# SinOncology/BreakID

Measured on AMD Instinct MI355X. Metric: M reads/s clustered+split-scanned, higher is better.
Workload: dtype int32/u8 (+f64 sd replay)

## Files before the change

### breakid_amd/csrc/api.hip

```cpp
#include <algorithm>
#include <cmath>
#include <limits>
#include <cstring>
#include <numeric>

#include "bk_common.h"
#include "prims.h"
#include "stream.h"
#include "join.h"
#include "cluster.h"
#include "bp.h"
#include "normal.h"
#include "genotype.h"
#include "clip.h"
#include "junction.h"
#include "evidence.h"
#include "unique.h"
#include "consensus.h"
#include "jfit.h"
#include "locsim.h"
#include "coverage.h"
#include "context.h"
#include "frame.h"
#include "link.h"
// ... 2250 lines not shown
int bk_debug_scan(bk_ctx *ctx, int elem_bytes, const void *in, uint64_t n, int in_place, void *out)
{
  return guarded(ctx, [&] {
    if (elem_bytes != 4 && elem_bytes != 8) throw bk_error(BK_ERR_ARG, "bk_debug_scan: elem_bytes must be 4 or 8");
    if (!out || (n && !in)) throw bk_error(BK_ERR_ARG, "bk_debug_scan: null argument");
    auto run = [&](auto zero) {
      using T = decltype(zero);
      T *d_in = ctx->dbg_in.as<T>(n + 1);
      T *d_out = in_place ? d_in : ctx->dbg_out.as<T>(n + 1);
      HIP_CHECK(hipMemsetAsync(d_out, 0xA5, (n + 1) * sizeof(T), ctx->st));
      if (n) HIP_CHECK(hipMemcpyAsync(d_in, in, n * sizeof(T), hipMemcpyHostToDevice, ctx->st));
      prims::exclusive_scan<T>(d_in, d_out, n, ctx->dbg_radix.scan_tmp, ctx->st);
      HIP_CHECK(hipMemcpyAsync(out, d_out, (n + 1) * sizeof(T), hipMemcpyDeviceToHost, ctx->st));
      HIP_CHECK(hipStreamSynchronize(ctx->st));
    };
    if (elem_bytes == 4)
      run(uint32_t(0));
    else
      run(uint64_t(0));
  });
}

int bk_debug_radix_sort(bk_ctx *ctx, const uint64_t *keys, const uint32_t *vals, uint64_t n, int begin_bit, int end_bit, uint64_t *keys_out, uint32_t *vals_out)
{
  return guarded(ctx, [&] {
    if (n && (!keys || !vals || !keys_out || !vals_out)) throw bk_error(BK_ERR_ARG, "bk_debug_radix_sort: null argument");
    if (begin_bit < 0 || end_bit > 64) throw bk_error(BK_ERR_ARG, "bk_debug_radix_sort: bits outside [0, 64]");
    prims::radix_check_count(n);
    if (!n) return;
    prims::RadixBufs &rb = ctx->dbg_radix;
    uint64_t *dk = ctx->dbg_in.as<uint64_t>(n);
    uint32_t *dv = ctx->dbg_vals.as<uint32_t>(n);
    HIP_CHECK(hipMemsetAsync(rb.keys_alt.as<uint64_t>(n), 0xA5, n * 8, ctx->st));
    HIP_CHECK(hipMemsetAsync(rb.vals_alt.as<uint32_t>(n), 0xA5, n * 4, ctx->st));
    HIP_CHECK(hipMemcpyAsync(dk, keys, n * 8, hipMemcpyHostToDevice, ctx->st));
    HIP_CHECK(hipMemcpyAsync(dv, vals, n * 4, hipMemcpyHostToDevice, ctx->st));
    uint64_t *ko = nullptr;
    uint32_t *vo = nullptr;
    prims::radix_sort_pairs(dk, dv, n, begin_bit, end_bit, rb, ctx->st, &ko, &vo);
    HIP_CHECK(hipMemcpyAsync(keys_out, ko, n * 8, hipMemcpyDeviceToHost, ctx->st));
    HIP_CHECK(hipMemcpyAsync(vals_out, vo, n * 4, hipMemcpyDeviceToHost, ctx->st));
    HIP_CHECK(hipStreamSynchronize(ctx->st));
  });
}

int bk_debug_prims_info(uint64_t out[4])
{
  if (!out) return BK_ERR_ARG;
  out[0] = prims::BLOCK;
  out[1] = prims::SCAN_TILE;
  out[2] = prims::SCAN_ONE_MAX;
  out[3] = prims::RS_TILE;
  return BK_OK;
}

int bk_sort_forms(bk_ctx *ctx, uint64_t out[3])
{
  return guarded(ctx, [&] {
    if (!out) throw bk_error(BK_ERR_ARG, "bk_sort_forms: null output");
    ctx->stage.sort_forms(out);
  });
}

int bk_debug_ahc(bk_ctx *ctx, const uint32_t *x, const uint32_t *y, uint32_t n, double w, uint32_t *idx_out, int32_t *cluster_out, uint32_t *n_out)
{
  return guarded(ctx, [&] {
    if (!x || !y || !idx_out || !cluster_out || !n_out) throw bk_error(BK_ERR_ARG, "bk_debug_ahc: null argument");
    std::vector<bk_pair> hp(n);
    for (uint32_t i = 0; i < n; ++i)
    {
      memset(&hp[i], 0, sizeof(bk_pair));
      hp[i].x = x[i];
      hp[i].y = y[i];
    }
    DevBuf dp, dcl;
    PairList L;
    L.n = n;
    L.ng = 1;
    std::vector<uint32_t> iota(n), gof(n, 0);
    std::iota(iota.begin(), iota.end(), 0u);
    uint64_t goff[2] = {0, n};
    HIP_CHECK(hipMemcpy(dp.as<bk_pair>(n + 1), hp.data(), n * sizeof(bk_pair), hipMemcpyHostToDevice));
    HIP_CHECK(hipMemcpy(L.idx.as<uint32_t>(n + 1), iota.data(), n * 4, hipMemcpyHostToDevice));
    HIP_CHECK(hipMemcpy(L.gof.as<uint32_t>(n + 1), gof.data(), n * 4, hipMemcpyHostToDevice));
    HIP_CHECK(hipMemcpy(L.goff.as<uint64_t>(2), goff, 16, hipMemcpyHostToDevice));
    ahc_cluster_all(dp.get<bk_pair>(), L, w, dcl, ctx->stage.ab, ctx->stage.cb(), ctx->st);
    *n_out = (uint32_t) L.n;
    if (L.n)
    {
      HIP_CHECK(hipMemcpyAsync(idx_out, L.idx.get<uint32_t>(), L.n * 4, hipMemcpyDeviceToHost, ctx->st));
      HIP_CHECK(hipMemcpyAsync(cluster_out, dcl.get<uint32_t>(), L.n * 4, hipMemcpyDeviceToHost, ctx->st));
    }
    HIP_CHECK(hipStreamSynchronize(ctx->st));
  });
}

}

namespace
{
struct FeedLink
{
  int device = 0, mapq_min = 20;
  bk_ctx *ctx = nullptr;
  int rc = BK_OK;
  std::string err;
  uint64_t done = 0;
  bool prepared = false, overflow = false;
  hipEvent_t t0 = nullptr, t1 = nullptr;
  template <class F> void guard(F &&f)
  {
    if (rc != BK_OK) return;
    try
    {
      f();
    }
    catch (const bk_error &e)
    {
      rc = e.code;
      err = e.msg;
    }
  }
};
void link_header(void *u, int nt, const char *const *names, const uint32_t *lens)
{
  FeedLink *L = (FeedLink *) u;
  if (L->ctx || L->rc != BK_OK) return;
  L->rc = bk_init(L->device, lens, names, nt, &L->ctx);
  if (L->rc != BK_OK) L->err = bk_last_error(nullptr);
}
void link_reset(void *u)
{
  FeedLink *L = (FeedLink *) u;
  L->guard([&] {
    if (L->ctx) HIP_CHECK(hipStreamSynchronize(L->ctx->st));
    L->done = 0;
    L->prepared = false;
    L->overflow = false;
  });
}
void link_before_move(void *u)
{
  FeedLink *L = (FeedLink *) u;
  L->guard([&] {
    if (L->ctx) HIP_CHECK(hipStreamSynchronize(L->ctx->st));
  });
}
void link_chunk(void *u, const bk_soa *cols, uint64_t n_ready, uint64_t n_est, hipEvent_t ready)
{
  FeedLink *L = (FeedLink *) u;
  L->guard([&] {
    bk_ctx *c = L->ctx;
    if (!c || n_ready < (uint64_t) STREAM_V + 1) return;
    c->rec = *cols;
    c->have_records = true;
    c->mapq_min = L->mapq_min;
    if (!L->prepared)
    {
      stream_prepare(c, n_est + n_est / 4);
      L->prepared = true;
    }
    const uint64_t lim = (n_ready - 1) / STREAM_V * STREAM_V;
    if (lim <= L->done) return;
    HIP_CHECK(hipStreamWaitEvent(c->st, ready, 0));
    StreamArgs a = stream_args(c, lim);
    a.q_begin = L->done / STREAM_V;
    launch_stream(a, c->st);
    L->done = lim;
  });
}
}


extern "C" {

int bk_bam_decode_device_ctx(const char *path, int device, int mapq_min, bk_bam_dev **bam_out, bk_ctx **ctx_out, int *n_targets, const char *const **names,
                             const uint32_t **lens, char *err, size_t errlen)
{
  auto fail = [&](int code, const std::string &m) {
    if (err && errlen) snprintf(err, errlen, "%s", m.c_str());
    return code;
  };
  if (!path || !bam_out || !ctx_out) return fail(BK_ERR_ARG, "bk_bam_decode_device_ctx: null argument");
  *bam_out = nullptr;
  *ctx_out = nullptr;
  FeedLink L;
  L.device = device;
  L.mapq_min = mapq_min;
  FeedConsumer fc;
  fc.user = &L;
  fc.on_header = link_header;
  fc.on_chunk = link_chunk;
  fc.before_move = link_before_move;
  fc.on_reset = link_reset;
  bk_soa cols;
  bk_bam_dev *bam = nullptr;
  int rc = bam_decode_device_impl(path, device, &bam, &cols, n_targets, names, lens, err, errlen, &fc);
  if (rc == BK_OK && L.rc != BK_OK) rc = fail(L.rc, L.err);
  if (rc == BK_OK && !L.ctx) rc = fail(BK_ERR_IO, "bk_bam_decode_device_ctx: no header");
  if (rc != BK_OK)
  {
    if (L.ctx) bk_free(L.ctx);
    if (bam) bk_bam_dev_free(bam);
    return rc;
  }
  bk_ctx *c = L.ctx;
  rc = guarded(c, [&] {
    const uint64_t done = L.prepared ? L.done : 0;
    c->stream_done = c->stats_done = c->clustered = false;
    c->rec = cols;
    c->have_records = true;
    c->mapq_min = mapq_min;
    c->rec_base = 0;
    bool ok = false;
    if (L.prepared)
    {
      Scope s(c, "k_stream", 39ull * cols.n + 4ull * cols.n_cigar_words);
      StreamArgs a = stream_args(c, cols.n);
      a.q_begin = done / STREAM_V;
      launch_stream(a, c->st);
      ok = stream_finish(c);
    }
    if (ok)
      stream_rare_path(c);
    else
      run_stream(c);
    if (bk_debug("feed"))
      fprintf(stderr, "[feed/stream] stream pass %s: %llu of %llu records went through k_stream while the file was still arriving\n", ok ? "overlapped" : "after the feed",
              (unsigned long long) (ok ? done : 0), (unsigned long long) cols.n);
  });
  if (rc != BK_OK)
  {
    fail(rc, c->err);
    bk_free(c);
    bk_bam_dev_free(bam);
    return rc;
  }
  *bam_out = bam;
  *ctx_out = c;
  return BK_OK;
}

int bk_group_stats(bk_ctx *ctx, const bk_group_stat **out, uint32_t *n_groups)
{
  return guarded(ctx, [&] {
    if (!out || !n_groups) throw bk_error(BK_ERR_ARG, "bk_group_stats: null output");
    if (!ctx->clustered) throw bk_error(BK_ERR_ARG, "bk_group_stats: call bk_mask_and_cluster (and bk_cluster_summary) first");
    const uint32_t ng = ctx->jr.n_groups;
    std::vector<uint64_t> iso(ng + 1, 0), clu(ng + 1, 0);
    std::vector<uint32_t> kmax(ng + 1, 0);
    if (ng)
    {
      HIP_CHECK(hipMemcpyAsync(iso.data(), ctx->stage.iso_goff.get<uint64_t>(), ((uint64_t) ng + 1) * 8, hipMemcpyDeviceToHost, ctx->st));
      HIP_CHECK(hipMemcpyAsync(clu.data(), ctx->stage.list.goff.get<uint64_t>(), ((uint64_t) ng + 1) * 8, hipMemcpyDeviceToHost, ctx->st));
      if (ctx->stage.list.n && ctx->bb.kmax.p) HIP_CHECK(hipMemcpyAsync(kmax.data(), ctx->bb.kmax.get<uint32_t>(), (uint64_t) ng * 4, hipMemcpyDeviceToHost, ctx->st));
      HIP_CHECK(hipStreamSynchronize(ctx->st));
    }
    ctx->f_gstats.assign(ng, bk_group_stat{});
    for (uint32_t l = 0; l < ng; ++l)
    {
      const uint32_t g = ctx->lex_to_num[l];
      bk_group_stat &o = ctx->f_gstats[l];
      const uint32_t k = ctx->gkey_host[g];
      o.p1_tid = (int32_t) (k / (uint32_t) (ctx->nt + 1)) - 1;
      o.p2_tid = (int32_t) (k % (uint32_t) (ctx->nt + 1)) - 1;
      o.n_scan = ctx->gstart_host[g + 1] - ctx->gstart_host[g];
      o.n_isolated_removed = iso[g + 1] - iso[g];
      o.n_clustered = clu[g + 1] - clu[g];
      o.cluster_id_end = o.n_clustered ? kmax[g] : 0;
      o.ordinal = ctx->glex_host[g];
    }
    *out = ctx->f_gstats.data();
    *n_groups = ng;
  });
}

int bk_debug_points_groups(bk_ctx *ctx, int mode, const uint32_t *x, const uint32_t *y, const uint64_t *group_off, uint32_t n_groups, double w, uint32_t *idx_out,
                           int32_t *cluster_out, uint64_t *goff_out, uint32_t *n_out)
{
  return guarded(ctx, [&] {
    if (!group_off || !idx_out || !n_out || mode < 0 || mode > 2) throw bk_error(BK_ERR_ARG, "bk_debug_points_groups: bad argument");
    if (group_off[0] != 0) throw bk_error(BK_ERR_ARG, "bk_debug_points_groups: group_off[0] must be 0");
    for (uint32_t g = 0; g < n_groups; ++g)
      if (group_off[g + 1] < group_off[g]) throw bk_error(BK_ERR_ARG, "bk_debug_points_groups: group_off must ascend");
    const uint64_t n = group_off[n_groups];
    if (n >= (1ull << 31) || (n && (!x || !y))) throw bk_error(BK_ERR_ARG, "bk_debug_points_groups: bad argument");
    std::vector<bk_pair> hp(n);
    std::vector<uint32_t> gof(n);
    for (uint32_t g = 0; g < n_groups; ++g)
      for (uint64_t i = group_off[g]; i < group_off[g + 1]; ++i)
      {
        memset(&hp[i], 0, sizeof(bk_pair));
        hp[i].x = x[i];
        hp[i].y = y[i];
        gof[i] = g;
      }
    DevBuf dp, dcl, dgof, dgoff;
    PairList L;
    const size_t goff_bytes = ((size_t) n_groups + 1) * 8;
    if (n) HIP_CHECK(hipMemcpy(dp.as<bk_pair>(n + 1), hp.data(), n * sizeof(bk_pair), hipMemcpyHostToDevice));
    if (n) HIP_CHECK(hipMemcpy(dgof.as<uint32_t>(n + 1), gof.data(), n * 4, hipMemcpyHostToDevice));
    HIP_CHECK(hipMemcpy(dgoff.as<uint64_t>((uint64_t) n_groups + 1), group_off, goff_bytes, hipMemcpyHostToDevice));
    const bk_pair *pairs = dp.as<bk_pair>(n + 1);
    if (mode == 1)
      remove_isolated_all(pairs, dgof.get<uint32_t>(), dgoff.get<uint64_t>(), n_groups, n, w, L, ctx->stage.cb(), ctx->st);
    else
    {
      L.n = n;
      L.ng = n_groups;
      std::vector<uint32_t> iota(n);
      std::iota(iota.begin(), iota.end(), 0u);
      uint32_t *lidx = L.idx.as<uint32_t>(n + 1), *lgof = L.gof.as<uint32_t>(n + 1);
      if (n) HIP_CHECK(hipMemcpy(lidx, iota.data(), n * 4, hipMemcpyHostToDevice));
      if (n) HIP_CHECK(hipMemcpy(lgof, gof.data(), n * 4, hipMemcpyHostToDevice));
      HIP_CHECK(hipMemcpy(L.goff.as<uint64_t>((uint64_t) n_groups + 1), group_off, goff_bytes, hipMemcpyHostToDevice));
      if (mode == 0)
        debug_mask_list(pairs, L, (long) w, ctx->stage.cb(), ctx->st);
      else
        fast_cluster_all(pairs, L, w, dcl, ctx->stage.cb(), ctx->st);
    }
    if (L.n > 2 * n) throw bk_error(BK_ERR_LIMIT, "bk_debug_points_groups: the list grew beyond 2 n entries");
    *n_out = (uint32_t) L.n;
    if (L.n)
    {
      HIP_CHECK(hipMemcpyAsync(idx_out, L.idx.get<uint32_t>(), L.n * 4, hipMemcpyDeviceToHost, ctx->st));
      if (mode == 2 && cluster_out) HIP_CHECK(hipMemcpyAsync(cluster_out, dcl.get<uint32_t>(), L.n * 4, hipMemcpyDeviceToHost, ctx->st));
    }
    if (goff_out)
    {
      if (n)
        HIP_CHECK(hipMemcpyAsync(goff_out, L.goff.get<uint64_t>(), goff_bytes, hipMemcpyDeviceToHost, ctx->st));
      else
        memset(goff_out, 0, goff_bytes);
    }
    HIP_CHECK(hipStreamSynchronize(ctx->st));
  });
}

int bk_debug_points(bk_ctx *ctx, int mode, const uint32_t *x, const uint32_t *y, uint32_t n, double w, uint32_t *idx_out, int32_t *cluster_out, uint32_t *n_out)
{
  const uint64_t goff[2] = {0, n};
  return bk_debug_points_groups(ctx, mode, x, y, goff, 1, w, idx_out, cluster_out, nullptr, n_out);
}

int bk_debug_cluster_info(uint64_t out[2])
{
  if (!out) return BK_ERR_ARG;
  out[0] = FW_TILE;
  out[1] = FW_LEVELS;
  return BK_OK;
}

int bk_debug_cigar(bk_ctx *ctx, uint32_t n, const uint8_t *kind, const uint32_t *c1_off, const uint8_t *c1, const uint32_t *c2_off, const uint8_t *c2, const int32_t *e,
                   int32_t *out6)
{
  return guarded(ctx, [&] {
    if (!n) return;
    if (!kind || !c1_off || !c1 || !c2_off || !c2 || !e || !out6) throw bk_error(BK_ERR_ARG, "bk_debug_cigar: null argument");
    DevBuf dk, d1o, d1, d2o, d2, de, dout;
    HIP_CHECK(hipMemcpy(dk.as<uint8_t>(n), kind, n, hipMemcpyHostToDevice));
    HIP_CHECK(hipMemcpy(d1o.as<uint32_t>(n + 1), c1_off, (n + 1) * 4, hipMemcpyHostToDevice));
    HIP_CHECK(hipMemcpy(d1.as<uint8_t>(c1_off[n] + 16), c1, c1_off[n], hipMemcpyHostToDevice));
    HIP_CHECK(hipMemcpy(d2o.as<uint32_t>(n + 1), c2_off, (n + 1) * 4, hipMemcpyHostToDevice));
    HIP_CHECK(hipMemcpy(d2.as<uint8_t>(c2_off[n] + 16), c2, c2_off[n], hipMemcpyHostToDevice));
    HIP_CHECK(hipMemcpy(de.as<int32_t>(n), e, n * 4, hipMemcpyHostToDevice));
    int32_t *o = dout.as<int32_t>(6ull * n);
    debug_cigar(dk.get<uint8_t>(), d1o.get<uint32_t>(), d1.get<uint8_t>(), d2o.get<uint32_t>(), d2.get<uint8_t>(), de.get<int32_t>(), n, o, ctx->st);
    HIP_CHECK(hipMemcpyAsync(out6, o, 24ull * n, hipMemcpyDeviceToHost, ctx->st));
    HIP_CHECK(hipStreamSynchronize(ctx->st));
  });
}

int bk_debug_vote(bk_ctx *ctx, const bk_split *side1, uint32_t n1, const bk_split *side2, uint32_t n2, int32_t p1_tid, int32_t p2_tid, int32_t *out3)
{
  return guarded(ctx, [&] {
    if ((n1 && !side1) || (n2 && !side2) || !out3) throw bk_error(BK_ERR_ARG, "bk_debug_vote: null argument");
    const uint32_t pos1 = 100000, pos2 = 300000;
    std::vector<bk_split> t;
    auto put = [&](const bk_split *src, uint32_t n, int32_t tid, uint32_t pos, uint64_t salt) {
      for (uint32_t i = 0; i < n + 2; ++i)
      {
        bk_split s;
        if (i < n)
          s = src[i];
        else
        {
          memset(&s, 0, sizeof s);
          s.qhash = 0xD00D000000000000ull + salt + i;
          s.prim_chr = s.sec_chr = -7;
        }
        s.tid = tid;
        s.pos = (int32_t) pos;
        s.endpos = (int32_t) pos + 50;
        t.push_back(s);
      }
    };
    put(side1, n1, p1_tid, pos1, 0);
    put(side2, n2, p2_tid, pos2, 1000);
    std::stable_sort(t.begin(), t.end(), [](const bk_split &a, const bk_split &b) { return (uint32_t) a.tid != (uint32_t) b.tid ? (uint32_t) a.tid < (uint32_t) b.tid : a.pos < b.pos; });
    for (size_t i = 0; i < t.size(); ++i) t[i].rec = i;
    bk_cluster c;
    memset(&c, 0, sizeof c);
    c.p1_tid = p1_tid;
    c.p2_tid = p2_tid;
    c.p1_mean = pos1 + 10;
    c.p2_mean = pos2 + 10;
    c.p1_exact = 0xFFFFFFFFu;
    c.p2_exact = -1;
    DevBuf dt, dc, dcov;
    HIP_CHECK(hipMemcpy(dt.as<bk_split>(t.size() + 1), t.data(), t.size() * sizeof(bk_split), hipMemcpyHostToDevice));
    HIP_CHECK(hipMemcpy(dc.as<bk_cluster>(2), &c, sizeof c, hipMemcpyHostToDevice));
    const uint32_t cov[2] = {5, 5};
    HIP_CHECK(hipMemcpy(dcov.as<uint32_t>(4), cov, 8, hipMemcpyHostToDevice));
    bp_vote(dt.get<bk_split>(), t.size(), dc.get<bk_cluster>(), 1, 1000.0, 200, dcov.get<uint32_t>(), ctx->d_hdr.get<int32_t>(), ctx->bb, ctx->st);
    uint32_t voted = 0;
    HIP_CHECK(hipMemcpyAsync(&voted, ctx->bb.voted.get<uint32_t>(), 4, hipMemcpyDeviceToHost, ctx->st));
    HIP_CHECK(hipMemcpyAsync(&c, dc.get<bk_cluster>(), sizeof c, hipMemcpyDeviceToHost, ctx->st));
    HIP_CHECK(hipStreamSynchronize(ctx->st));
    out3[0] = voted ? (int32_t) c.p1_exact : -1;
    out3[1] = voted ? c.p2_exact : -1;
    out3[2] = voted ? (int32_t) c.n_sr : 0;
  });
}

int bk_debug_region(bk_ctx *ctx, int32_t tid, uint32_t start, uint32_t end, uint64_t depth_pos, bk_split *out, uint32_t cap, uint32_t *n_out, uint32_t *cov_out,
                    uint32_t *depth_out)
{
  return guarded(ctx, [&] {
    if (!ctx->stream_done) run_stream(ctx);
    ensure_splits_sorted(ctx);
    DevBuf dout, dres;
    bk_split *o = dout.as<bk_split>((uint64_t) cap + 1);
    uint32_t *res = dres.as<uint32_t>(4);
    debug_region(rec_view(ctx), ctx->d_split.get<bk_split>(), ctx->hc.n_split, tid, start, end, (int) ctx->hc.max_span, depth_pos, o, cap, res, ctx->st);
    uint32_t h[4] = {0, 0, 0, 0};
    HIP_CHECK(hipMemcpyAsync(h, res, 16, hipMemcpyDeviceToHost, ctx->st));
    HIP_CHECK(hipStreamSynchronize(ctx->st));
    const uint32_t n = h[0] < cap ? h[0] : cap;
    if (n && out) HIP_CHECK(hipMemcpy(out, o, n * sizeof(bk_split), hipMemcpyDeviceToHost));
    if (n_out) *n_out = h[0];
    if (cov_out) *cov_out = h[1];
    if (depth_out) *depth_out = h[2];
  });
}

int bk_timing_enable(bk_ctx *ctx, int on)
{
  return guarded(ctx, [&] {
    ctx->timing = on != 0;
    for (auto &t : ctx->timers)
    {
      if (t.a) (void) hipEventDestroy(t.a);
      if (t.b) (void) hipEventDestroy(t.b);
    }
    ctx->timers.clear();
  });
}

int bk_timing(bk_ctx *ctx, const char *const **names, const float **ms, const uint64_t **bytes, int *n)
{
  return guarded(ctx, [&] {
    HIP_CHECK(hipStreamSynchronize(ctx->st));
    Timing &t = ctx->tout;
    t.names.clear(); t.ms.clear(); t.bytes.clear(); t.touched.clear(); t.cnames.clear();
    for (auto &s : ctx->timers)
    {
      float v = 0;
      HIP_CHECK(hipEventElapsedTime(&v, s.a, s.b));
      t.names.push_back(s.name);
      t.ms.push_back(v);
      t.bytes.push_back(s.bytes);
      t.touched.push_back(s.touched);
    }
    for (auto &s : t.names) t.cnames.push_back(s.c_str());
    if (names) *names = t.cnames.data();
    if (ms) *ms = t.ms.data();
    if (bytes) *bytes = t.bytes.data();
    if (n) *n = (int) t.names.size();
  });
}

int bk_timing_touched(bk_ctx *ctx, const uint64_t **touched, int *n)
{
  return guarded(ctx, [&] {
    if (touched) *touched = ctx->tout.touched.data();
    if (n) *n = (int) ctx->tout.touched.size();
  });
}

}
```

### breakid_amd/csrc/cluster.h

```cpp
#pragma once
#include "bk_common.h"
#include "prims.h"
#include "sortemu.h"

constexpr uint32_t FW_TILE = 1024, FW_LEVELS = 10;
static_assert((1ull << FW_LEVELS) >= FW_TILE, "k_fw_exit / k_fw_mark: FW_LEVELS rounds of doubling must cover a tile of one-element windows");
static_assert(FW_LEVELS < 32 && FW_TILE <= 1024 && FW_TILE < 0xFFFFu, "FW_TILE is a workgroup size and its positions are uint16");

struct PairList
{
  uint64_t n = 0;
  uint32_t ng = 0;
  DevBuf idx;
  DevBuf gof;
  DevBuf goff;
  uint64_t total(hipStream_t st) const;
};

struct ClusterBufs
{
  std::vector<uint32_t> heavy_x, heavy_y;
  bool observe = false;
  uint64_t max_group_bound = 0;
  DevBuf key, perm, tmp, cnt, off, off2, idx2, gof2, goff2, jump, mark, apos, kid, kprev2, k1, k2, pk, knum, clfull, small, scan_tmp;
  SortEmuBufs se;
  prims::RadixBufs radix;
};

void remove_isolated_all(const bk_pair *pairs, const uint32_t *gof0, const uint64_t *gstart, uint32_t ng, uint64_t n, double w, PairList &L, ClusterBufs &b, hipStream_t st,
                         const uint32_t *drop_group = nullptr);
void remove_isolated_begin(const bk_pair *pairs, const uint32_t *gof0, const uint64_t *gstart, uint32_t ng, uint64_t n, double w, PairList &L, ClusterBufs &b, hipStream_t st,
                           const uint32_t *drop_group = nullptr, const uint64_t *gstart_host = nullptr, const uint8_t *keep_host = nullptr);
void remove_isolated_end(const bk_pair *pairs, PairList &L, ClusterBufs &b, hipStream_t st);
void list_subset_ranges(const PairList &src, const uint64_t *src_goff_host, const uint8_t *keep_host, PairList &dst, hipStream_t st);
void drop_small_groups(PairList &L, ClusterBufs &b, hipStream_t st);
void fast_cluster_all(const bk_pair *pairs, PairList &L, double w, DevBuf &cluster_out, ClusterBufs &b, hipStream_t st);
void merge_lists_many(const PairList *const *lists, const uint32_t *const *cls, int K, PairList &out, DevBuf *cl_out, hipStream_t st);
void debug_mask_list(const bk_pair *pairs, PairList &L, long dist, ClusterBufs &b, hipStream_t st);
```

### breakid_amd/csrc/cluster.hip

```cpp
#include "bk_common.h"
#include "prims.h"
#include "sortemu.h"
#include "cluster.h"

namespace
{
constexpr uint32_t END = 0xFFFFFFFFu;

__global__ __launch_bounds__(256) void k_iota(uint32_t *__restrict__ a, uint64_t n)
{
  uint64_t i = (uint64_t) blockIdx.x * blockDim.x + threadIdx.x;
  if (i < n) a[i] = (uint32_t) i;
}
__global__ __launch_bounds__(256) void k_gather_key(const bk_pair *__restrict__ pairs, const uint32_t *__restrict__ idx, uint64_t n, int use_y, uint32_t *__restrict__ key)
{
  uint64_t p = (uint64_t) blockIdx.x * blockDim.x + threadIdx.x;
  if (p < n) key[p] = use_y ? pairs[idx[p]].y : pairs[idx[p]].x;
}
__global__ __launch_bounds__(256) void k_gather_u32(const uint32_t *__restrict__ src, const uint32_t *__restrict__ perm, uint64_t n, uint32_t *__restrict__ dst)
{
  uint64_t p = (uint64_t) blockIdx.x * blockDim.x + threadIdx.x;
  if (p < n) dst[p] = src[perm[p]];
}

__device__ __forceinline__ long absdiff(uint32_t a, uint32_t b)
{
  long d = (long) (int32_t) (a - b);
  return d < 0 ? -d : d;
}

__global__ __launch_bounds__(256) void k_mask_count(const bk_pair *__restrict__ pairs, const uint32_t *__restrict__ idx, const uint32_t *__restrict__ gof,
                                                    const uint64_t *__restrict__ goff, uint64_t n, long dist, uint32_t *__restrict__ cnt)
{
  uint64_t p = (uint64_t) blockIdx.x * blockDim.x + threadIdx.x;
  if (p >= n) return;
  uint32_t g = gof[p];
  uint64_t gs = goff[g], ge = goff[g + 1];
  uint64_t np = ge - gs, i = p - gs;
  uint32_t c = 0;
  if (np >= 3 && i >= 1 && i + 1 < np)
  {
    const bk_pair a = pairs[idx[p]], l = pairs[idx[p - 1]], r = pairs[idx[p + 1]];
    long ll = absdiff(l.x, a.x), lr = absdiff(r.x, a.x);
    long Lx = ll < lr ? ll : lr;
    ll = absdiff(l.y, a.y);
    lr = absdiff(r.y, a.y);
    long Ly = ll < lr ? ll : lr;
    if (!(Lx > dist || Ly > dist)) c += 1;
    if (i == 1)
    {
      long fx = absdiff(a.x, r.x), fy = absdiff(a.y, r.y);
      if (!(fx > dist || fy > dist)) c += 1;
    }
  }
  cnt[p] = c;
}

__global__ __launch_bounds__(256) void k_expand(const uint32_t *__restrict__ cnt, const uint32_t *__restrict__ off, const uint32_t *__restrict__ idx,
                                                const uint32_t *__restrict__ gof, uint64_t n, uint32_t *__restrict__ oidx, uint32_t *__restrict__ ogof)
{
  uint64_t p = (uint64_t) blockIdx.x * blockDim.x + threadIdx.x;
  if (p >= n) return;
  uint32_t c = cnt[p], o = off[p];
  for (uint32_t k = 0; k < c; ++k)
  {
    oidx[o + k] = idx[p];
    ogof[o + k] = gof[p];
  }
}
__global__ void k_new_goff(const uint32_t *__restrict__ off, const uint64_t *__restrict__ goff, uint32_t ng, uint64_t n, uint64_t *__restrict__ ogoff)
{
  uint32_t g = blockIdx.x * blockDim.x + threadIdx.x;
  if (g > ng) return;
  uint64_t s = g < ng ? goff[g] : n;
  ogoff[g] = off[s];
}

__global__ __launch_bounds__(256) void k_fast_next(const uint32_t *__restrict__ key, const uint32_t *__restrict__ gof, const uint64_t *__restrict__ goff, uint64_t n, double w,
                                                   uint32_t *__restrict__ nxt)
{
  uint64_t p = (uint64_t) blockIdx.x * blockDim.x + threadIdx.x;
  if (p >= n) return;
  uint32_t g = gof[p];
  uint64_t ge = goff[g + 1];
  if (p + 1 >= ge)
  {
    nxt[p] = END;
    return;
  }
  double lim = (double) (long) key[p] + w;
  uint64_t lo = p + 1, hi = ge;
  while (lo < hi)
  {
    uint64_t m = (lo + hi) >> 1;
    if ((double) key[m] <= lim) lo = m + 1; else hi = m;
  }
  if (lo > ge - 1) lo = ge - 1;
  nxt[p] = (uint32_t) lo;
}
__global__ void k_mark_starts(const uint64_t *__restrict__ goff, uint32_t ng, uint32_t *__restrict__ mark)
{
  uint32_t g = blockIdx.x * blockDim.x + threadIdx.x;
  if (g >= ng) return;
  if (goff[g + 1] > goff[g]) mark[goff[g]] = 1;
}
__global__ __launch_bounds__(FW_TILE) void k_fw_exit(const uint32_t *__restrict__ nxt, uint64_t n, uint32_t *__restrict__ exitp)
{
  __shared__ uint32_t e[FW_TILE];
  const uint64_t t0 = (uint64_t) blockIdx.x * FW_TILE, p = t0 + threadIdx.x;
  const uint64_t tend = t0 + FW_TILE;
  e[threadIdx.x] = p < n ? nxt[p] : END;
  for (uint32_t r = 0; r < FW_LEVELS; ++r)
  {
    __syncthreads();
    const uint32_t v = e[threadIdx.x];
    if (v != END && v < tend) e[threadIdx.x] = e[v - t0];
  }
  __syncthreads();
  if (p < n) exitp[p] = e[threadIdx.x];
}
__global__ __launch_bounds__(64) void k_fw_chain(const uint64_t *__restrict__ goff, uint32_t ng, const uint32_t *__restrict__ exitp, uint32_t *__restrict__ mark)
{
  const uint32_t g = blockIdx.x * blockDim.x + threadIdx.x;
  if (g >= ng || goff[g + 1] <= goff[g]) return;
  uint32_t p = (uint32_t) goff[g];
  for (;;)
  {
    const uint32_t q = exitp[p];
    if (q == END) break;
    mark[q] = 1;
    p = q;
  }
}
__global__ __launch_bounds__(FW_TILE) void k_fw_mark(const uint32_t *__restrict__ nxt, uint64_t n, uint32_t *__restrict__ mark)
{
  __shared__ uint16_t j[FW_LEVELS][FW_TILE];
  __shared__ uint32_t m[FW_TILE];
  constexpr uint16_t OUT = 0xFFFFu;
  const uint64_t t0 = (uint64_t) blockIdx.x * FW_TILE, p = t0 + threadIdx.x;
  const uint32_t i = threadIdx.x;
  uint32_t v = p < n ? nxt[p] : END;
  j[0][i] = (v != END && v < t0 + FW_TILE) ? (uint16_t) (v - t0) : OUT;
  m[i] = p < n ? mark[p] : 0u;
  for (uint32_t k = 1; k < FW_LEVELS; ++k)
  {
    __syncthreads();
    const uint16_t a = j[k - 1][i];
    j[k][i] = a == OUT ? OUT : j[k - 1][a];
  }
  for (int k = FW_LEVELS - 1; k >= 0; --k)
  {
    __syncthreads();
    if (m[i])
    {
      const uint16_t t = j[k][i];
      if (t != OUT) m[t] = 1u;
    }
  }
  __syncthreads();
  if (p < n) mark[p] = m[i];
}

__global__ __launch_bounds__(256) void k_anchor_pos(const uint32_t *__restrict__ mark, const uint32_t *__restrict__ ascan, uint64_t n, uint32_t *__restrict__ apos)
{
  uint64_t p = (uint64_t) blockIdx.x * blockDim.x + threadIdx.x;
  if (p < n && mark[p]) apos[ascan[p]] = (uint32_t) p;
}
__global__ __launch_bounds__(256) void k_fast_keep(const uint32_t *__restrict__ mark, const uint32_t *__restrict__ ascan, const uint32_t *__restrict__ apos,
                                                   const uint32_t *__restrict__ nxt, uint64_t n, uint32_t *__restrict__ keep, uint32_t *__restrict__ kid)
{
  uint64_t p = (uint64_t) blockIdx.x * blockDim.x + threadIdx.x;
  if (p >= n) return;
  uint32_t ord = ascan[p] + mark[p] - 1;
  uint32_t a = apos[ord];
  uint32_t e = nxt[a];
  keep[p] = (e != END && e - a >= 2) ? 1u : 0u;
  kid[p] = ord;
}
__global__ __launch_bounds__(256) void k_compact3(const uint32_t *__restrict__ keep, const uint32_t *__restrict__ off, uint64_t n, const uint32_t *__restrict__ a0,
                                                  const uint32_t *__restrict__ a1, const uint32_t *__restrict__ a2, const uint32_t *__restrict__ a3, uint32_t *__restrict__ o0,
                                                  uint32_t *__restrict__ o1, uint32_t *__restrict__ o2, uint32_t *__restrict__ o3)
{
  uint64_t p = (uint64_t) blockIdx.x * blockDim.x + threadIdx.x;
  if (p >= n || !keep[p]) return;
  uint32_t o = off[p];
  o0[o] = a0[p];
  if (a1) o1[o] = a1[p];
  if (a2) o2[o] = a2[p];
  if (a3) o3[o] = a3[p];
}
__global__ __launch_bounds__(256) void k_pack_k(const uint32_t *__restrict__ k1, const uint32_t *__restrict__ k2, uint64_t n, int kbits, uint64_t *__restrict__ key, uint32_t *__restrict__ val)
{
  uint64_t p = (uint64_t) blockIdx.x * blockDim.x + threadIdx.x;
  if (p >= n) return;
  key[p] = ((uint64_t) k2[p] << kbits) | k1[p];
  val[p] = (uint32_t) p;
}
__global__ __launch_bounds__(256) void k_run_flag(const uint64_t *__restrict__ key, uint64_t n, uint32_t *__restrict__ flag)
{
  uint64_t p = (uint64_t) blockIdx.x * blockDim.x + threadIdx.x;
  if (p < n) flag[p] = (p == 0 || key[p] != key[p - 1]) ? 1u : 0u;
}
__global__ __launch_bounds__(256) void k_uid_stats(const uint32_t *__restrict__ flag, const uint32_t *__restrict__ fscan, const uint32_t *__restrict__ val, uint64_t n,
                                                   uint32_t *__restrict__ uid_of_elem, uint32_t *__restrict__ ustart, uint32_t *__restrict__ uminpos)
{
  uint64_t q = (uint64_t) blockIdx.x * blockDim.x + threadIdx.x;
  if (q >= n) return;
  const uint32_t f = flag[q];
  uint32_t u = fscan[q] + f - 1;
  uint32_t e = val[q];
  uid_of_elem[e] = u;
  if (f)
  {
    ustart[u] = (uint32_t) q;
    uminpos[u] = e;
  }
  if (q == n - 1) ustart[u + 1] = (uint32_t) n;
}
__global__ __launch_bounds__(256) void k_first_flag(const uint32_t *__restrict__ uid, const uint32_t *__restrict__ ustart, const uint32_t *__restrict__ uminpos, uint64_t n,
                                                    uint32_t *__restrict__ keep, uint32_t *__restrict__ first)
{
  uint64_t p = (uint64_t) blockIdx.x * blockDim.x + threadIdx.x;
  if (p >= n) return;
  uint32_t u = uid[p];
  uint32_t k = ustart[u + 1] - ustart[u] >= 2 ? 1u : 0u;
  keep[p] = k;
  first[p] = (k && uminpos[u] == (uint32_t) p) ? 1u : 0u;
}
__global__ __launch_bounds__(256) void k_knum(const uint32_t *__restrict__ first, const uint32_t *__restrict__ fscan, const uint32_t *__restrict__ uid,
                                              const uint32_t *__restrict__ gof, const uint64_t *__restrict__ goff, uint64_t n, uint32_t *__restrict__ knum)
{
  uint64_t p = (uint64_t) blockIdx.x * blockDim.x + threadIdx.x;
  if (p >= n || !first[p]) return;
  uint64_t gs = goff[gof[p]];
  knum[uid[p]] = fscan[p] - fscan[gs] + 1;
}
__global__ __launch_bounds__(256) void k_cluster_of(const uint32_t *__restrict__ uid, const uint32_t *__restrict__ knum, const uint32_t *__restrict__ keep, uint64_t n,
                                                    uint32_t *__restrict__ cl)
{
  uint64_t p = (uint64_t) blockIdx.x * blockDim.x + threadIdx.x;
  if (p < n) cl[p] = keep[p] ? knum[uid[p]] : 0u;
}
__global__ void k_group_small(const uint64_t *__restrict__ goff, uint32_t ng, uint32_t *__restrict__ small)
{
  uint32_t g = blockIdx.x * blockDim.x + threadIdx.x;
  if (g < ng) small[g] = (goff[g + 1] - goff[g]) < 2 ? 1u : 0u;
}
__global__ __launch_bounds__(256) void k_drop_small(const uint32_t *__restrict__ gof, const uint32_t *__restrict__ small, uint64_t n, uint32_t *__restrict__ keep)
{
  uint64_t p = (uint64_t) blockIdx.x * blockDim.x + threadIdx.x;
  if (p < n) keep[p] = small[gof[p]] ? 0u : 1u;
}
}

uint64_t PairList::total(hipStream_t st) const
{
  uint64_t t = 0;
  if (ng == 0) return 0;
  HIP_CHECK(hipMemcpyAsync(&t, goff.get<uint64_t>() + ng, 8, hipMemcpyDeviceToHost, st));
  HIP_CHECK(hipStreamSynchronize(st));
  return t;
}

static inline unsigned nb(uint64_t n) { return cdiv(n ? n : 1, 256); }
static void filter_groups(PairList &L, const uint32_t *drop, ClusterBufs &b, hipStream_t st);

static void sort_list(const bk_pair *pairs, PairList &L, int use_y, uint32_t **extra, int n_extra, ClusterBufs &b, hipStream_t st)
{
  if (L.n == 0) return;
  uint32_t *key = b.key.as<uint32_t>(L.n), *perm = b.perm.as<uint32_t>(L.n);
  hipLaunchKernelGGL(k_gather_key, dim3(nb(L.n)), dim3(256), 0, st, pairs, L.idx.get<uint32_t>(), L.n, use_y, key);
  hipLaunchKernelGGL(k_iota, dim3(nb(L.n)), dim3(256), 0, st, perm, L.n);
  b.se.heavy = b.observe ? (use_y ? &b.heavy_y : &b.heavy_x) : nullptr;
  std_sort_groups(key, perm, L.gof.get<uint32_t>(), L.goff.get<uint64_t>(), L.ng, L.n, b.se, st);
  b.se.heavy = nullptr;
  uint32_t *tmp = b.tmp.as<uint32_t>(L.n);
  auto apply = [&](uint32_t *arr) {
    hipLaunchKernelGGL(k_gather_u32, dim3(nb(L.n)), dim3(256), 0, st, arr, perm, L.n, tmp);
    HIP_CHECK(hipMemcpyAsync(arr, tmp, L.n * 4, hipMemcpyDeviceToDevice, st));
  };
  apply(L.idx.get<uint32_t>());
  for (int k = 0; k < n_extra; ++k) apply(extra[k]);
}

static void mask_list(const bk_pair *pairs, PairList &L, long dist, ClusterBufs &b, hipStream_t st)
{
  if (L.n == 0) return;
  uint32_t *cnt = b.cnt.as<uint32_t>(L.n + 1);
  hipLaunchKernelGGL(k_mask_count, dim3(nb(L.n)), dim3(256), 0, st, pairs, L.idx.get<uint32_t>(), L.gof.get<uint32_t>(), L.goff.get<uint64_t>(), L.n, dist, cnt);
  uint32_t *off = b.off.as<uint32_t>(L.n + 1);
  prims::exclusive_scan<uint32_t>(cnt, off, L.n, b.scan_tmp, st);
  uint32_t total = 0;
  HIP_CHECK(hipMemcpyAsync(&total, off + L.n, 4, hipMemcpyDeviceToHost, st));
  HIP_CHECK(hipStreamSynchronize(st));
  uint32_t *oidx = b.idx2.as<uint32_t>((uint64_t) total + 1), *ogof = b.gof2.as<uint32_t>((uint64_t) total + 1);
  uint64_t *ogoff = b.goff2.as<uint64_t>((uint64_t) L.ng + 1);
  hipLaunchKernelGGL(k_expand, dim3(nb(L.n)), dim3(256), 0, st, cnt, off, L.idx.get<uint32_t>(), L.gof.get<uint32_t>(), L.n, oidx, ogof);
  hipLaunchKernelGGL(k_new_goff, dim3(cdiv(L.ng + 1, 256)), dim3(256), 0, st, off, L.goff.get<uint64_t>(), L.ng, L.n, ogoff);
  std::swap(L.idx, b.idx2);
  std::swap(L.gof, b.gof2);
  std::swap(L.goff, b.goff2);
  L.n = total;
}

void remove_isolated_all(const bk_pair *pairs, const uint32_t *gof0, const uint64_t *gstart, uint32_t ng, uint64_t n, double w, PairList &L, ClusterBufs &b, hipStream_t st,
                         const uint32_t *drop_group)
{
  remove_isolated_begin(pairs, gof0, gstart, ng, n, w, L, b, st, drop_group, nullptr, nullptr);
  remove_isolated_end(pairs, L, b, st);
}

void remove_isolated_end(const bk_pair *pairs, PairList &L, ClusterBufs &b, hipStream_t st)
{
  if (L.n == 0 || L.ng == 0) return;
  sort_list(pairs, L, 0, nullptr, 0, b, st);
}

namespace
{
__global__ __launch_bounds__(256) void k_subset_list(const uint64_t *__restrict__ gstart, const uint64_t *__restrict__ goff, uint32_t ng, uint64_t n_list,
                                                     uint32_t *__restrict__ idx, uint32_t *__restrict__ gof)
{
  const uint64_t p = (uint64_t) blockIdx.x * blockDim.x + threadIdx.x;
  if (p >= n_list) return;
  uint32_t lo = 0, hi = ng;
  while (hi - lo > 1)
  {
    const uint32_t m = (lo + hi) >> 1;
    if (goff[m] <= p) lo = m; else hi = m;
  }
  idx[p] = (uint32_t) (gstart[lo] + (p - goff[lo]));
  gof[p] = lo;
}
}
namespace
{
__global__ __launch_bounds__(256) void k_subset_of_list(const uint32_t *__restrict__ src_idx, const uint64_t *__restrict__ src_goff, const uint64_t *__restrict__ goff, uint32_t ng,
                                                        uint64_t n_list, uint32_t *__restrict__ idx, uint32_t *__restrict__ gof)
{
  const uint64_t p = (uint64_t) blockIdx.x * blockDim.x + threadIdx.x;
  if (p >= n_list) return;
  uint32_t lo = 0, hi = ng;
  while (hi - lo > 1)
  {
    const uint32_t m = (lo + hi) >> 1;
    if (goff[m] <= p) lo = m; else hi = m;
  }
  idx[p] = src_idx[src_goff[lo] + (p - goff[lo])];
  gof[p] = lo;
}
}
void list_subset_ranges(const PairList &src, const uint64_t *src_goff_host, const uint8_t *keep_host, PairList &dst, hipStream_t st)
{
  const uint32_t ng = src.ng;
  std::vector<uint64_t> goff((size_t) ng + 1, 0);
  for (uint32_t g = 0; g < ng; ++g) goff[g + 1] = goff[g] + (keep_host[g] ? src_goff_host[g + 1] - src_goff_host[g] : 0);
  dst.n = goff[ng];
  dst.ng = ng;
  uint32_t *idx = dst.idx.as<uint32_t>(dst.n + 1), *gof = dst.gof.as<uint32_t>(dst.n + 1);
  uint64_t *dgoff = dst.goff.as<uint64_t>((uint64_t) ng + 1);
  HIP_CHECK(hipMemcpyAsync(dgoff, goff.data(), ((size_t) ng + 1) * 8, hipMemcpyHostToDevice, st));
  HIP_CHECK(hipStreamSynchronize(st));
  if (dst.n) hipLaunchKernelGGL(k_subset_of_list, dim3(nb(dst.n)), dim3(256), 0, st, src.idx.get<uint32_t>(), src.goff.get<uint64_t>(), dgoff, ng, dst.n, idx, gof);
}

void list_of_groups(const uint64_t *gstart_dev, const uint64_t *gstart_host, const uint8_t *keep_host, uint32_t ng, PairList &L, hipStream_t st)
{
  std::vector<uint64_t> goff((size_t) ng + 1, 0);
  for (uint32_t g = 0; g < ng; ++g) goff[g + 1] = goff[g] + (keep_host[g] ? gstart_host[g + 1] - gstart_host[g] : 0);
  L.n = goff[ng];
  L.ng = ng;
  uint32_t *idx = L.idx.as<uint32_t>(L.n + 1), *gof = L.gof.as<uint32_t>(L.n + 1);
  uint64_t *dgoff = L.goff.as<uint64_t>((uint64_t) ng + 1);
  HIP_CHECK(hipMemcpyAsync(dgoff, goff.data(), ((size_t) ng + 1) * 8, hipMemcpyHostToDevice, st));
  HIP_CHECK(hipStreamSynchronize(st));
  if (L.n) hipLaunchKernelGGL(k_subset_list, dim3(nb(L.n)), dim3(256), 0, st, gstart_dev, dgoff, ng, L.n, idx, gof);
}

void remove_isolated_begin(const bk_pair *pairs, const uint32_t *gof0, const uint64_t *gstart, uint32_t ng, uint64_t n, double w, PairList &L, ClusterBufs &b, hipStream_t st,
                           const uint32_t *drop_group, const uint64_t *gstart_host, const uint8_t *keep_host)
{
  if (gstart_host && keep_host)
  {
    if (n == 0 || ng == 0)
    {
      L.n = 0;
      L.ng = ng;
      (void) L.idx.as<uint32_t>(1);
      (void) L.gof.as<uint32_t>(1);
      (void) L.goff.as<uint64_t>((uint64_t) ng + 1);
      return;
    }
    list_of_groups(gstart, gstart_host, keep_host, ng, L, st);
  }
  else
  {
    L.n = n;
    L.ng = ng;
    uint32_t *idx = L.idx.as<uint32_t>(n + 1);
    uint32_t *gof = L.gof.as<uint32_t>(n + 1);
    uint64_t *goff = L.goff.as<uint64_t>((uint64_t) ng + 1);
    if (n == 0 || ng == 0) return;
    hipLaunchKernelGGL(k_iota, dim3(nb(n)), dim3(256), 0, st, idx, n);
    HIP_CHECK(hipMemcpyAsync(gof, gof0, n * 4, hipMemcpyDeviceToDevice, st));
    HIP_CHECK(hipMemcpyAsync(goff, gstart, ((uint64_t) ng + 1) * 8, hipMemcpyDeviceToDevice, st));
    if (drop_group) filter_groups(L, drop_group, b, st);
  }
  if (L.n == 0) return;
  const long dist = (long) w;
  sort_list(pairs, L, 0, nullptr, 0, b, st);
  mask_list(pairs, L, dist, b, st);
  sort_list(pairs, L, 1, nullptr, 0, b, st);
  mask_list(pairs, L, dist, b, st);
}

static void fast_pass(const bk_pair *pairs, PairList &L, int use_y, double w, DevBuf &k_prev, DevBuf &k_new, ClusterBufs &b, hipStream_t st)
{
  if (L.n == 0) return;
  const uint64_t n = L.n;
  uint32_t *key = b.key.as<uint32_t>(n);
  hipLaunchKernelGGL(k_gather_key, dim3(nb(n)), dim3(256), 0, st, pairs, L.idx.get<uint32_t>(), n, use_y, key);
  uint32_t *jump = b.jump.as<uint32_t>(n * 2ull);
  hipLaunchKernelGGL(k_fast_next, dim3(nb(n)), dim3(256), 0, st, key, L.gof.get<uint32_t>(), L.goff.get<uint64_t>(), n, w, jump);
  uint32_t *mark = b.mark.as<uint32_t>(n + 1);
  HIP_CHECK(hipMemsetAsync(mark, 0, (n + 1) * 4, st));
  hipLaunchKernelGGL(k_mark_starts, dim3(cdiv(L.ng, 256)), dim3(256), 0, st, L.goff.get<uint64_t>(), L.ng, mark);
  {
    uint32_t *exitp = jump + n;
    const unsigned tiles = (unsigned) cdiv(n, FW_TILE);
    hipLaunchKernelGGL(k_fw_exit, dim3(tiles), dim3(FW_TILE), 0, st, jump, n, exitp);
    hipLaunchKernelGGL(k_fw_chain, dim3(cdiv(L.ng, 64)), dim3(64), 0, st, L.goff.get<uint64_t>(), L.ng, exitp, mark);
    hipLaunchKernelGGL(k_fw_mark, dim3(tiles), dim3(FW_TILE), 0, st, jump, n, mark);
  }
  uint32_t *ascan = b.off.as<uint32_t>(n + 1);
  prims::exclusive_scan<uint32_t>(mark, ascan, n, b.scan_tmp, st);
  uint32_t *apos = b.apos.as<uint32_t>(n + 1);
  hipLaunchKernelGGL(k_anchor_pos, dim3(nb(n)), dim3(256), 0, st, mark, ascan, n, apos);
  uint32_t *keep = b.cnt.as<uint32_t>(n + 1), *kid = b.kid.as<uint32_t>(n + 1);
  hipLaunchKernelGGL(k_fast_keep, dim3(nb(n)), dim3(256), 0, st, mark, ascan, apos, jump, n, keep, kid);
  uint32_t *off = b.off2.as<uint32_t>(n + 1);
  prims::exclusive_scan<uint32_t>(keep, off, n, b.scan_tmp, st);
  uint32_t total = 0;
  HIP_CHECK(hipMemcpyAsync(&total, off + n, 4, hipMemcpyDeviceToHost, st));
  HIP_CHECK(hipStreamSynchronize(st));
  uint32_t *oidx = b.idx2.as<uint32_t>((uint64_t) total + 1), *ogof = b.gof2.as<uint32_t>((uint64_t) total + 1);
  uint32_t *okn = k_new.as<uint32_t>((uint64_t) total + 1);
  uint32_t *okp = k_prev.p ? b.kprev2.as<uint32_t>((uint64_t) total + 1) : nullptr;
  uint64_t *ogoff = b.goff2.as<uint64_t>((uint64_t) L.ng + 1);
  hipLaunchKernelGGL(k_compact3, dim3(nb(n)), dim3(256), 0, st, keep, off, n, L.idx.get<uint32_t>(), L.gof.get<uint32_t>(), kid, k_prev.get<uint32_t>(), oidx, ogof, okn, okp);
  hipLaunchKernelGGL(k_new_goff, dim3(cdiv(L.ng + 1, 256)), dim3(256), 0, st, off, L.goff.get<uint64_t>(), L.ng, n, ogoff);
  std::swap(L.idx, b.idx2);
  std::swap(L.gof, b.gof2);
  std::swap(L.goff, b.goff2);
  if (k_prev.p) std::swap(k_prev, b.kprev2);
  L.n = total;
}

static void filter_groups(PairList &L, const uint32_t *drop, ClusterBufs &b, hipStream_t st)
{
  if (L.n == 0) return;
  uint32_t *keep = b.cnt.as<uint32_t>(L.n + 1), *off = b.off.as<uint32_t>(L.n + 1);
  hipLaunchKernelGGL(k_drop_small, dim3(nb(L.n)), dim3(256), 0, st, L.gof.get<uint32_t>(), drop, L.n, keep);
  prims::exclusive_scan<uint32_t>(keep, off, L.n, b.scan_tmp, st);
  uint32_t total = 0;
  HIP_CHECK(hipMemcpyAsync(&total, off + L.n, 4, hipMemcpyDeviceToHost, st));
  HIP_CHECK(hipStreamSynchronize(st));
  if (total != L.n)
  {
    uint32_t *oidx = b.idx2.as<uint32_t>((uint64_t) total + 1), *ogof = b.gof2.as<uint32_t>((uint64_t) total + 1);
    uint64_t *ogoff = b.goff2.as<uint64_t>((uint64_t) L.ng + 1);
    hipLaunchKernelGGL(k_compact3, dim3(nb(L.n)), dim3(256), 0, st, keep, off, L.n, L.idx.get<uint32_t>(), L.gof.get<uint32_t>(), (const uint32_t *) nullptr,
                       (const uint32_t *) nullptr, oidx, ogof, (uint32_t *) nullptr, (uint32_t *) nullptr);
    hipLaunchKernelGGL(k_new_goff, dim3(cdiv(L.ng + 1, 256)), dim3(256), 0, st, off, L.goff.get<uint64_t>(), L.ng, L.n, ogoff);
    std::swap(L.idx, b.idx2);
    std::swap(L.gof, b.gof2);
    std::swap(L.goff, b.goff2);
    L.n = total;
  }
}

void drop_small_groups(PairList &L, ClusterBufs &b, hipStream_t st)
{
  if (L.n == 0) return;
  uint32_t *small = b.small.as<uint32_t>((uint64_t) L.ng + 1);
  hipLaunchKernelGGL(k_group_small, dim3(cdiv(L.ng, 256)), dim3(256), 0, st, L.goff.get<uint64_t>(), L.ng, small);
  filter_groups(L, small, b, st);
}

void fast_cluster_all(const bk_pair *pairs, PairList &L, double w, DevBuf &cluster_out, ClusterBufs &b, hipStream_t st)
{
  drop_small_groups(L, b, st);
  DevBuf none;
  const uint64_t n_first = L.n;
  fast_pass(pairs, L, 0, w, none, b.k1, b, st);
  {
    uint32_t *extra[1] = {b.k1.get<uint32_t>()};
    sort_list(pairs, L, 1, extra, L.n ? 1 : 0, b, st);
  }
  fast_pass(pairs, L, 1, w, b.k1, b.k2, b, st);
  {
    uint32_t *extra[2] = {b.k1.get<uint32_t>(), b.k2.get<uint32_t>()};
    sort_list(pairs, L, 0, extra, L.n ? 2 : 0, b, st);
  }
  const uint64_t n = L.n;
  uint32_t *cl = cluster_out.as<uint32_t>(n + 1);
  if (n == 0) return;
  uint64_t *pk = b.pk.as<uint64_t>(n);
  uint32_t *pv = b.perm.as<uint32_t>(n);
  int kbits = 1;
  while (kbits < 32 && (n_first >> kbits) != 0) ++kbits;
  hipLaunchKernelGGL(k_pack_k, dim3(nb(n)), dim3(256), 0, st, b.k1.get<uint32_t>(), b.k2.get<uint32_t>(), n, kbits, pk, pv);
  uint64_t *ks;
  uint32_t *vs;
  prims::radix_sort_pairs(pk, pv, n, 0, std::min(64, 2 * kbits), b.radix, st, &ks, &vs);
  uint32_t *flag = b.cnt.as<uint32_t>(n + 1), *fscan = b.off.as<uint32_t>(n + 1);
  hipLaunchKernelGGL(k_run_flag, dim3(nb(n)), dim3(256), 0, st, ks, n, flag);
  prims::exclusive_scan<uint32_t>(flag, fscan, n, b.scan_tmp, st);
  uint32_t *uid = b.kid.as<uint32_t>(n + 1), *ucount = b.mark.as<uint32_t>(n + 2), *uminpos = b.apos.as<uint32_t>(n + 1);
  hipLaunchKernelGGL(k_uid_stats, dim3(nb(n)), dim3(256), 0, st, flag, fscan, vs, n, uid, ucount, uminpos);
  uint32_t *keep = b.off2.as<uint32_t>(n + 1), *first = b.key.as<uint32_t>(n + 1);
  hipLaunchKernelGGL(k_first_flag, dim3(nb(n)), dim3(256), 0, st, uid, ucount, uminpos, n, keep, first);
  uint32_t *fs2 = b.tmp.as<uint32_t>(n + 1);
  prims::exclusive_scan<uint32_t>(first, fs2, n, b.scan_tmp, st);
  uint32_t *knum = b.knum.as<uint32_t>(n + 1);
  hipLaunchKernelGGL(k_knum, dim3(nb(n)), dim3(256), 0, st, first, fs2, uid, L.gof.get<uint32_t>(), L.goff.get<uint64_t>(), n, knum);
  uint32_t *clfull = b.clfull.as<uint32_t>(n + 1);
  hipLaunchKernelGGL(k_cluster_of, dim3(nb(n)), dim3(256), 0, st, uid, knum, keep, n, clfull);
  uint32_t *off = b.off.as<uint32_t>(n + 1);
  prims::exclusive_scan<uint32_t>(keep, off, n, b.scan_tmp, st);
  uint32_t total = 0;
  HIP_CHECK(hipMemcpyAsync(&total, off + n, 4, hipMemcpyDeviceToHost, st));
  HIP_CHECK(hipStreamSynchronize(st));
  uint32_t *oidx = b.idx2.as<uint32_t>((uint64_t) total + 1), *ogof = b.gof2.as<uint32_t>((uint64_t) total + 1);
  uint64_t *ogoff = b.goff2.as<uint64_t>((uint64_t) L.ng + 1);
  cl = cluster_out.as<uint32_t>((uint64_t) total + 1);
  hipLaunchKernelGGL(k_compact3, dim3(nb(n)), dim3(256), 0, st, keep, off, n, L.idx.get<uint32_t>(), L.gof.get<uint32_t>(), clfull, (const uint32_t *) nullptr, oidx, ogof, cl,
                     (uint32_t *) nullptr);
  hipLaunchKernelGGL(k_new_goff, dim3(cdiv(L.ng + 1, 256)), dim3(256), 0, st, off, L.goff.get<uint64_t>(), L.ng, n, ogoff);
  std::swap(L.idx, b.idx2);
  std::swap(L.gof, b.gof2);
  std::swap(L.goff, b.goff2);
  L.n = total;
}

void debug_mask_list(const bk_pair *pairs, PairList &L, long dist, ClusterBufs &b, hipStream_t st) { mask_list(pairs, L, dist, b, st); }

namespace
{
__global__ __launch_bounds__(256) void k_merge_goff(const uint64_t *__restrict__ b, uint32_t ng, uint64_t *__restrict__ out)
{
  uint32_t g = blockIdx.x * blockDim.x + threadIdx.x;
  if (g <= ng) out[g] += b[g];
}
__global__ __launch_bounds__(256) void k_merge_copy(const uint32_t *__restrict__ idx, const uint32_t *__restrict__ gof, const uint32_t *__restrict__ cl, const uint64_t *__restrict__ goff,
                                                    uint64_t n, const uint64_t *__restrict__ mgoff, uint32_t *__restrict__ oidx, uint32_t *__restrict__ ogof, uint32_t *__restrict__ ocl)
{
  uint64_t p = (uint64_t) blockIdx.x * blockDim.x + threadIdx.x;
  if (p >= n) return;
  const uint32_t g = gof[p];
  const uint64_t d = mgoff[g] + (p - goff[g]);
  oidx[d] = idx[p];
  ogof[d] = g;
  if (cl) ocl[d] = cl[p];
}
}

void merge_lists_many(const PairList *const *lists, const uint32_t *const *cls, int K, PairList &out, DevBuf *cl_out, hipStream_t st)
{
  const uint32_t ng = lists[0]->ng;
  out.ng = ng;
  out.n = 0;
  for (int l = 0; l < K; ++l) out.n += lists[l]->n;
  uint32_t *oidx = out.idx.as<uint32_t>(out.n + 1), *ogof = out.gof.as<uint32_t>(out.n + 1);
  uint64_t *ogoff = out.goff.as<uint64_t>((uint64_t) ng + 1);
  uint32_t *ocl = cl_out ? cl_out->as<uint32_t>(out.n + 1) : nullptr;
  HIP_CHECK(hipMemsetAsync(ogoff, 0, ((size_t) ng + 1) * 8, st));
  for (int l = 0; l < K; ++l) hipLaunchKernelGGL(k_merge_goff, dim3(cdiv(ng + 1, 256)), dim3(256), 0, st, lists[l]->goff.get<uint64_t>(), ng, ogoff);
  for (int l = 0; l < K; ++l)
  {
    const PairList &A = *lists[l];
    if (A.n) hipLaunchKernelGGL(k_merge_copy, dim3(nb(A.n)), dim3(256), 0, st, A.idx.get<uint32_t>(), A.gof.get<uint32_t>(), cls ? cls[l] : nullptr, A.goff.get<uint64_t>(), A.n, ogoff, oidx, ogof, ocl);
  }
}
```

### breakid_amd/csrc/lanes.h

```cpp
#pragma once
#include <functional>
#include <memory>

#include "join.h"
#include "cluster.h"
#include "ahc.h"

void stage_set_hw_queues(int n);

struct StageInput
{
  int device;
  hipStream_t st;
  const JoinResult &jr;
  const std::vector<uint64_t> &gstart_host;
  const std::vector<uint8_t> &own_groups;
  std::function<void(const char *name, const std::function<void()> &body)> timed;
};

struct ClusterStage
{
  SortService svc;
  std::vector<hipEvent_t> svc_probe;
  int svc_late = 0;
  bool svc_refused = false;
  struct Lane
  {
    ClusterBufs cb;
    PairList list, iso;
    DevBuf d_cluster;
    hipStream_t st = nullptr;
    ~Lane()
    {
      if (st) (void) hipStreamDestroy(st);
    }
  };
  std::vector<std::unique_ptr<Lane>> lanes;
  ClusterBufs &cb() { return lanes[0]->cb; }
  AhcBufs ab;
  PairList list;
  DevBuf d_cluster, iso_idx, iso_goff;
  uint64_t iso_n = 0;
  PairList lane_mid, lane_iso_m;
  DevBuf d_drop;

  ClusterStage() { lanes.emplace_back(new Lane()); }
  void run(const StageInput &in, double w, int fast);
  void sort_forms(uint64_t out[3]) const;
  void debug_sort(int device, hipStream_t st, uint32_t *key, uint32_t *idx, const uint32_t *gof, const uint64_t *goff, uint32_t ng, uint64_t n, uint64_t max_group);
};
```

### breakid_amd/csrc/lanes.hip

```cpp
#include <algorithm>
#include <atomic>
#include <chrono>
#include <cmath>
#include <cstdio>
#include <numeric>
#include <thread>
#include <dirent.h>

#include "lanes.h"

static int g_hw_queues_at_init = 0;
void stage_set_hw_queues(int n) { g_hw_queues_at_init = n; }

static bool sort_service_on()
{
  static const bool on = !(getenv("BREAKID_SORT_SERVICE") && atoi(getenv("BREAKID_SORT_SERVICE")) == 0);
  return on;
}
constexpr int LANE_STREAMS_MAX = 4;
constexpr int SVC_STAGE_QUEUES = LANE_STREAMS_MAX + 3;
static bool lane_service(int fast) { return sort_service_on() && fast && g_hw_queues_at_init >= SVC_STAGE_QUEUES; }
static int stage_queues() { return std::max(1, g_hw_queues_at_init - 1); }
static int lanes_wanted(bool svc)
{
  const char *env = getenv("BREAKID_GROUP_LANES");
  static const int want_svc = env ? atoi(env) : 12;
  if (svc) return want_svc < 1 ? 1 : (want_svc > 26 ? 26 : want_svc);
  static const int want = env ? atoi(env) : std::min(4, stage_queues());
  return want < 1 ? 1 : (want > 26 ? 26 : want);
}
static bool lanes_apply(const StageInput &in, int fast)
{
  static const uint64_t min_pairs = getenv("BREAKID_LANES_MIN_PAIRS") ? strtoull(getenv("BREAKID_LANES_MIN_PAIRS"), nullptr, 10) : (1ull << 20);
  uint32_t large = 0;
  const uint64_t big = std::max<uint64_t>(2, min_pairs >> 6);
  for (uint32_t g = 0; g < in.jr.n_groups && g + 1 < in.gstart_host.size(); ++g) large += in.gstart_host[g + 1] - in.gstart_host[g] >= big ? 1u : 0u;
  const bool yes = lanes_wanted(lane_service(fast)) >= 2 && fast && in.jr.n_groups >= 4 && in.jr.n_pairs >= min_pairs && large >= 2;
  if (yes)
  {
    static bool told = false;
    const int K = lanes_wanted(lane_service(fast));
    if (!told && !lane_service(fast) && K > stage_queues() && bk_debug("lanes"))
    {
      told = true;
      fprintf(stderr, "[breakid] GPU_MAX_HW_QUEUES=%d: the lanes of chromosome-pair groups (bk_mask_and_cluster) and their heap kernels will share hardware queues "
                        "(BREAKID_GROUP_LANES=1: one pass)\n", g_hw_queues_at_init);
    }
  }
  return yes;
}

__global__ void k_svc_probe() {}
static int kfd_compute_queues(int device)
{
  char bus[64] = {0};
  if (hipDeviceGetPCIBusId(bus, (int) sizeof bus, device) != hipSuccess) return -1;
  unsigned dom = 0, b = 0, d = 0, f = 0;
  if (sscanf(bus, "%x:%x:%x.%x", &dom, &b, &d, &f) != 4) return -1;
  const unsigned long want_loc = (b << 8) | (d << 3) | f;
  auto read_file = [](const std::string &path, std::string &out) {
    FILE *fp = fopen(path.c_str(), "r");
    if (!fp) return false;
    char buf[4096];
    const size_t n = fread(buf, 1, sizeof buf - 1, fp);
    fclose(fp);
    buf[n] = 0;
    out = buf;
    return true;
  };
  auto list_dir = [](const std::string &path, std::vector<std::string> &names) {
    DIR *dp = opendir(path.c_str());
    if (!dp) return false;
    while (dirent *e = readdir(dp))
      if (e->d_name[0] != '.') names.push_back(e->d_name);
    closedir(dp);
    return true;
  };
  unsigned long gpu_id = 0;
  {
    std::vector<std::string> nodes;
    if (!list_dir("/sys/class/kfd/kfd/topology/nodes", nodes)) return -1;
    for (const std::string &n : nodes)
    {
      std::string props, id;
      const std::string base = "/sys/class/kfd/kfd/topology/nodes/" + n;
      if (!read_file(base + "/properties", props) || !read_file(base + "/gpu_id", id)) continue;
      unsigned long loc = ~0ul, domain = ~0ul;
      size_t p = props.find("location_id ");
      if (p != std::string::npos) loc = strtoul(props.c_str() + p + 12, nullptr, 10);
      p = props.find("domain ");
      if (p != std::string::npos) domain = strtoul(props.c_str() + p + 7, nullptr, 10);
      if (loc == want_loc && (domain == ~0ul || domain == dom) && strtoul(id.c_str(), nullptr, 10) != 0) gpu_id = strtoul(id.c_str(), nullptr, 10);
    }
  }
  if (!gpu_id) return -1;
  std::vector<std::string> procs;
  if (!list_dir("/sys/class/kfd/kfd/proc", procs)) return -1;
  int total = 0;
  for (const std::string &pid : procs)
  {
    std::vector<std::string> qs;
    const std::string qdir = "/sys/class/kfd/kfd/proc/" + pid + "/queues";
    if (!list_dir(qdir, qs)) continue;
    for (const std::string &q : qs)
    {
      std::string g, t;
      if (!read_file(qdir + "/" + q + "/gpuid", g) || !read_file(qdir + "/" + q + "/type", t)) continue;
      if (strtoul(g.c_str(), nullptr, 10) == gpu_id && strtoul(t.c_str(), nullptr, 10) == 0) ++total;
    }
  }
  return total;
}
constexpr int SVC_MAX_DEVICE_QUEUES = 24;
static std::mutex g_svc_device_m[64];
static void tell_no_service()
{
  static std::atomic<bool> told{false};
  if (!getenv("BREAKID_QUIET") && !told.exchange(true))
    fprintf(stderr, "[breakid] the resident sort service shares a hardware queue with a stream of its own stage (GPU_MAX_HW_QUEUES too low for the streams of this process), or other processes hold hardware queues on this device: sorting by launches instead\n");
}
struct SvcStage
{
  ClusterStage &cs;
  hipStream_t st;
  bool on;
  std::unique_lock<std::mutex> device_turn;
  SvcStage(ClusterStage &s, int device, hipStream_t st, bool want, uint64_t n_bound, uint64_t max_group, const std::vector<hipStream_t> &streams)
      : cs(s), st(st), on(want && sort_service_on() && !s.svc_refused)
  {
    if (on && device >= 0 && device < 64)
    {
      device_turn = std::unique_lock<std::mutex>(g_svc_device_m[device], std::try_to_lock);
      on = device_turn.owns_lock();
    }
    if (!on) return;
    const auto ts0 = std::chrono::steady_clock::now();
    cs.svc.start(n_bound, max_group + 2, st);
    const auto ts1 = std::chrono::steady_clock::now();
    int census;
    {
      static std::mutex cm;
      static std::chrono::steady_clock::time_point when[64];
      static int last[64];
      static bool have[64] = {};
      std::lock_guard<std::mutex> l(cm);
      const int d = device & 63;
      if (!have[d] || std::chrono::duration<double>(ts1 - when[d]).count() > 0.25)
      {
        last[d] = kfd_compute_queues(device);
        when[d] = std::chrono::steady_clock::now();
        have[d] = true;
      }
      census = last[d];
    }
    if (bk_debug("lanes"))
      fprintf(stderr, "[lanes] sort service started in %.3f ms; compute queues on the device (all processes): %d (counted in %.3f ms)\n", std::chrono::duration<double, std::milli>(ts1 - ts0).count(), census,
              std::chrono::duration<double, std::milli>(std::chrono::steady_clock::now() - ts1).count());
    const bool crowded = census > SVC_MAX_DEVICE_QUEUES;
    const bool behind = !crowded && !reachable(streams);
    const bool late = !crowded && !behind && !cs.svc.narrow_running(0.03);
    if (crowded || behind || late)
    {
      cs.svc.stop();
      on = false;
      if (crowded || behind || ++cs.svc_late >= 2) cs.svc_refused = true;
      device_turn.unlock();
      tell_no_service();
      return;
    }
    cs.svc_late = 0;
    set(&cs.svc);
  }
  bool reachable(const std::vector<hipStream_t> &streams)
  {
    while (cs.svc_probe.size() < streams.size())
    {
      hipEvent_t e;
      HIP_CHECK(hipEventCreateWithFlags(&e, hipEventDisableTiming));
      cs.svc_probe.push_back(e);
    }
    for (size_t k = 0; k < streams.size(); ++k)
    {
      hipLaunchKernelGGL(k_svc_probe, dim3(1), dim3(64), 0, streams[k]);
      HIP_CHECK(hipEventRecord(cs.svc_probe[k], streams[k]));
    }
    const auto t0 = std::chrono::steady_clock::now();
    auto since = [&] { return std::chrono::duration<double>(std::chrono::steady_clock::now() - t0).count(); };
    bool ok = true;
    for (size_t k = 0; k < streams.size() && ok; ++k)
      for (;;)
      {
        const hipError_t e = hipEventQuery(cs.svc_probe[k]);
        if (e == hipSuccess) break;
        if (e != hipErrorNotReady) throw bk_error(BK_ERR_HIP, std::string("sort service probe: ") + hipGetErrorString(e));
        if (since() > 0.05)
        {
          ok = false;
          break;
        }
      }
    const double took = since();
    if (bk_debug("lanes")) fprintf(stderr, "[lanes] sort service probe: %zu streams in %.3f ms%s\n", streams.size(), took * 1e3, ok ? "" : " (gave up)");
    return ok && took < 0.003;
  }
  void set(SortService *s)
  {
    for (auto &l : cs.lanes)
    {
      l->cb.se.svc = s;
      l->cb.se.svc_slot = 0xFFFFFFFFu;
    }
  }
  void finish()
  {
    if (!on) return;
    on = false;
    set(nullptr);
    hipError_t e = hipStreamSynchronize(st);
    for (auto &l : cs.lanes)
      if (l->st && e == hipSuccess) e = hipStreamSynchronize(l->st);
    cs.svc.stop();
    device_turn.unlock();
    if (e != hipSuccess) throw bk_error(BK_ERR_HIP, std::string("sort service: ") + hipGetErrorString(e));
  }
  ~SvcStage()
  {
    try
    {
      finish();
    }
    catch (const bk_error &)
    {
    }
  }
};

static void snapshot_list(const PairList &L, DevBuf &idx, DevBuf *gof, DevBuf &goff, hipStream_t st)
{
  uint32_t *ii = idx.as<uint32_t>(L.n + 1), *ig = gof ? gof->as<uint32_t>(L.n + 1) : nullptr;
  uint64_t *io = goff.as<uint64_t>((uint64_t) L.ng + 1);
  if (L.n) HIP_CHECK(hipMemcpyAsync(ii, L.idx.get<uint32_t>(), L.n * 4, hipMemcpyDeviceToDevice, st));
  if (L.n && ig) HIP_CHECK(hipMemcpyAsync(ig, L.gof.get<uint32_t>(), L.n * 4, hipMemcpyDeviceToDevice, st));
  if (L.ng) HIP_CHECK(hipMemcpyAsync(io, L.goff.get<uint64_t>(), ((uint64_t) L.ng + 1) * 8, hipMemcpyDeviceToDevice, st));
}
static void cluster_list(const bk_pair *pairs, PairList &L, double w, int fast, DevBuf &cl, ClusterBufs &cb, AhcBufs &ab, hipStream_t st)
{
  if (fast)
    fast_cluster_all(pairs, L, w, cl, cb, st);
  else
    ahc_cluster_all(pairs, L, w, cl, ab, cb, st);
}

using LanePlan = std::vector<int>;
static LanePlan plan_owned(const StageInput &in)
{
  const uint32_t ng = in.jr.n_groups;
  const bool owned_only = !in.own_groups.empty();
  if (owned_only && in.own_groups.size() != ng) throw bk_error(BK_ERR_ARG, "bk_shard_own_groups: group count changed");
  LanePlan p(ng, 0);
  for (uint32_t g = 0; owned_only && g < ng; ++g)
    if (!in.own_groups[g]) p[g] = -1;
  return p;
}
static LanePlan plan_blind(const StageInput &in, int K)
{
  const uint32_t ng = in.jr.n_groups;
  std::vector<uint32_t> order(ng);
  std::iota(order.begin(), order.end(), 0u);
  auto size_of = [&](uint32_t g) { return in.gstart_host[g + 1] - in.gstart_host[g]; };
  std::stable_sort(order.begin(), order.end(), [&](uint32_t a, uint32_t b) { return size_of(a) > size_of(b); });
  constexpr double wexp = 2.0;
  LanePlan p = plan_owned(in);
  std::vector<double> load(K, 0.0);
  for (uint32_t i = 0; i < ng; ++i)
  {
    const uint32_t g = order[i];
    if (p[g] < 0) continue;
    int l = 0;
    for (int k = 1; k < K; ++k)
      if (load[k] < load[l]) l = k;
    load[l] += std::pow((double) size_of(g), wexp);
    p[g] = l;
  }
  return p;
}
static LanePlan plan_observed(const std::vector<uint64_t> &sizes, const std::vector<uint32_t> &hx, const std::vector<uint32_t> &hy, int K)
{
  const uint32_t ng = (uint32_t) sizes.size();
  constexpr double per_pair = 0.001;
  auto heap_cost = [](uint32_t m) { return (double) m + (m > 40947u ? 1.0 * (double) (m - 40947u) : 0.0); };
  std::vector<uint32_t> order(ng);
  std::iota(order.begin(), order.end(), 0u);
  auto chain = [&](uint32_t g) { return heap_cost(hx[g]) + heap_cost(hy[g]); };
  std::stable_sort(order.begin(), order.end(), [&](uint32_t a, uint32_t b) {
    const double ca = chain(a), cb = chain(b);
    return ca != cb ? ca > cb : sizes[a] > sizes[b];
  });
  LanePlan p(ng, 0);
  std::vector<double> mx(K, 0.0), my(K, 0.0), pairs(K, 0.0);
  auto cost = [&](int l) { return mx[l] + my[l] + per_pair * pairs[l]; };
  for (uint32_t g : order)
  {
    int best = 0;
    double best_cost = 0;
    for (int l = 0; l < K; ++l)
    {
      const double c = std::max(mx[l], heap_cost(hx[g])) + std::max(my[l], heap_cost(hy[g])) + per_pair * (pairs[l] + (double) sizes[g]);
      if (l == 0 || c < best_cost || (c == best_cost && cost(l) < cost(best)))
      {
        best = l;
        best_cost = c;
      }
    }
    mx[best] = std::max(mx[best], heap_cost(hx[g]));
    my[best] = std::max(my[best], heap_cost(hy[g]));
    pairs[best] += (double) sizes[g];
    p[g] = best;
  }
  if (bk_debug("lanes"))
    for (int l = 0; l < K; ++l)
    {
      fprintf(stderr, "[lanes] lane %d: max heap x %.0f y %.0f, %.0f pairs, cost %.0f; heavy groups:", l, mx[l], my[l], pairs[l], cost(l));
      for (uint32_t g = 0; g < ng; ++g)
        if (p[g] == l && (hx[g] || hy[g])) fprintf(stderr, " %u(%u,%u)", g, hx[g], hy[g]);
      fprintf(stderr, "\n");
    }
  return p;
}
static uint32_t *upload_drop(const LanePlan &p, int K, DevBuf &buf, hipStream_t st)
{
  const size_t row = p.size() + 1;
  std::vector<uint32_t> drop((size_t) K * row, 0u);
  for (int l = 0; l < K; ++l)
    for (size_t g = 0; g + 1 < row; ++g) drop[(size_t) l * row + g] = p[g] == l ? 0u : 1u;
  uint32_t *d = buf.as<uint32_t>(drop.size() + 1);
  HIP_CHECK(hipMemcpyAsync(d, drop.data(), drop.size() * 4, hipMemcpyHostToDevice, st));
  HIP_CHECK(hipStreamSynchronize(st));
  return d;
}

static void group_lanes(ClusterStage &cs, const StageInput &in, double w, int fast)
{
  const uint32_t ng = in.jr.n_groups;
  static const bool dbg = bk_debug("lanes");
  auto make_lanes = [&](int K, int S) {
    while ((int) cs.lanes.size() < K)
    {
      cs.lanes.emplace_back(new ClusterStage::Lane());
      cs.lanes.back()->cb.max_group_bound = cs.cb().max_group_bound;
    }
    for (int k = 1; k < S; ++k)
      if (!cs.lanes[k]->st) HIP_CHECK(hipStreamCreateWithFlags(&cs.lanes[k]->st, hipStreamNonBlocking));
  };
  bool use_svc = sort_service_on() && fast;
  if (use_svc && !lane_service(fast))
  {
    use_svc = false;
    tell_no_service();
    if (bk_debug("lanes")) fprintf(stderr, "[lanes] %d hardware queues, the sort service needs %d: not started\n", g_hw_queues_at_init, SVC_STAGE_QUEUES);
  }
  int K = lanes_wanted(use_svc);
  int S = use_svc ? std::max(1, std::min(LANE_STREAMS_MAX, K)) : K;
  make_lanes(K, S);
  std::vector<hipStream_t> stage_streams{in.st};
  for (int k = 1; k < S; ++k) stage_streams.push_back(cs.lanes[k]->st);
  SvcStage svc_stage(cs, in.device, in.st, use_svc, in.jr.n_pairs + 2ull * ng + 4096, cs.cb().max_group_bound, stage_streams);
  if (use_svc && !svc_stage.on)
  {
    use_svc = false;
    K = lanes_wanted(false);
    S = K;
    make_lanes(K, S);
  }
  if (!use_svc && bk_debug("lanes"))
  {
    fprintf(stderr, "[lanes] launch path: %d lanes, 1 stream each, %d hardware queues\n", K, g_hw_queues_at_init);
    fprintf(stderr, "[lanes] sorts as task dispatches on the lane streams\n");
  }
  auto lane = [&](int l) -> ClusterStage::Lane & { return *cs.lanes[l]; };
  auto lane_st = [&](int l) { const int k = l % S; return k == 0 ? in.st : cs.lanes[k]->st; };
  uint32_t *drop_base = nullptr;
  auto lane_drop = [&](int l) { return drop_base + (size_t) l * ((size_t) ng + 1); };
  std::vector<std::vector<uint8_t>> keep(K, std::vector<uint8_t>(ng, 0));
  auto upload_plan = [&](const LanePlan &p) {
    for (int l = 0; l < K; ++l)
      for (uint32_t g = 0; g < ng; ++g) keep[l][g] = p[g] == l ? 1 : 0;
    drop_base = upload_drop(p, K, cs.d_drop, in.st);
  };
  auto in_lanes = [&](auto body) {
    std::vector<std::string> err(K);
    std::vector<int> code(K, BK_OK);
    const auto t_start = std::chrono::steady_clock::now();
    auto guarded_body = [&](int l) {
      try
      {
        body(l);
        HIP_CHECK(hipStreamSynchronize(lane_st(l)));
        if (dbg)
          fprintf(stderr, "[lanes] lane %d done after %.2f ms\n", l, std::chrono::duration<double, std::milli>(std::chrono::steady_clock::now() - t_start).count());
      }
      catch (const bk_error &e)
      {
        code[l] = e.code;
        err[l] = e.msg;
      }
    };
    std::vector<std::thread> th;
    for (int l = 1; l < K; ++l)
      th.emplace_back([&, l] {
        (void) hipSetDevice(in.device);
        guarded_body(l);
      });
    guarded_body(0);
    for (std::thread &t : th) t.join();
    for (int l = 0; l < K; ++l)
      if (code[l] != BK_OK) throw bk_error(code[l], err[l]);
  };
  auto merge_all = [&](PairList ClusterStage::Lane::*which, PairList &out, DevBuf *cl_out) {
    std::vector<const PairList *> ls(K);
    std::vector<const uint32_t *> cls(K);
    for (int l = 0; l < K; ++l)
    {
      ls[l] = &(lane(l).*which);
      cls[l] = lane(l).d_cluster.get<uint32_t>();
    }
    merge_lists_many(ls.data(), cl_out ? cls.data() : nullptr, K, out, cl_out, in.st);
  };
  const bk_pair *pairs = in.jr.pairs;
  auto mask_lane = [&](int l, bool observe) {
    ClusterBufs &cb = lane(l).cb;
    if (observe)
    {
      cb.heavy_x.assign(ng, 0u);
      cb.heavy_y.assign(ng, 0u);
      cb.observe = true;
      cb.se.heavy_all = false;
    }
    remove_isolated_begin(pairs, in.jr.gof, in.jr.gstart, ng, in.jr.n_pairs, w, lane(l).list, cb, lane_st(l), lane_drop(l), in.gstart_host.data(), keep[l].data());
    if (observe) cb.heavy_x.assign(ng, 0u);
    remove_isolated_end(pairs, lane(l).list, cb, lane_st(l));
    if (observe) cb.observe = false;
  };
  auto cluster_lane = [&](int l) {
    PairList &L = lane(l).list, &iso = lane(l).iso;
    iso.n = L.n;
    iso.ng = L.ng;
    snapshot_list(L, iso.idx, &iso.gof, iso.goff, lane_st(l));
    cluster_list(pairs, L, w, fast, lane(l).d_cluster, lane(l).cb, cs.ab, lane_st(l));
  };
  const auto tp0 = std::chrono::steady_clock::now();
  auto phase = [&](const char *what) {
    if (dbg) fprintf(stderr, "[lanes] %s at %.2f ms\n", what, std::chrono::duration<double, std::milli>(std::chrono::steady_clock::now() - tp0).count());
  };
  upload_plan(plan_blind(in, K));
  phase("plan uploaded");
  if (use_svc)
    in_lanes([&](int l) {
      mask_lane(l, false);
      cluster_lane(l);
    });
  else
  {
    in_lanes([&](int l) { mask_lane(l, true); });
    PairList &mid = cs.lane_mid;
    merge_all(&ClusterStage::Lane::list, mid, nullptr);
    std::vector<uint64_t> goff_h((size_t) ng + 1);
    HIP_CHECK(hipMemcpyAsync(goff_h.data(), mid.goff.get<uint64_t>(), ((size_t) ng + 1) * 8, hipMemcpyDeviceToHost, in.st));
    HIP_CHECK(hipStreamSynchronize(in.st));
    std::vector<uint64_t> sizes(ng);
    std::vector<uint32_t> hx(ng, 0u), hy(ng, 0u);
    for (uint32_t g = 0; g < ng; ++g) sizes[g] = goff_h[g + 1] - goff_h[g];
    for (int l = 0; l < K; ++l)
      for (uint32_t g = 0; g < ng; ++g)
      {
        hx[g] = std::max(hx[g], lane(l).cb.heavy_x[g]);
        hy[g] = std::max(hy[g], lane(l).cb.heavy_y[g]);
      }
    upload_plan(plan_observed(sizes, hx, hy, K));
    in_lanes([&](int l) {
      list_subset_ranges(mid, goff_h.data(), keep[l].data(), lane(l).list, lane_st(l));
      cluster_lane(l);
    });
  }
  phase("lanes done");
  svc_stage.finish();
  phase("service stopped");
  if (use_svc && bk_debug("lanes")) fprintf(stderr, "[svc] tasks: %u wide, %u narrow\n", cs.svc.stats[0], cs.svc.stats[1]);
  PairList &iso_m = cs.lane_iso_m;
  merge_all(&ClusterStage::Lane::iso, iso_m, nullptr);
  merge_all(&ClusterStage::Lane::list, cs.list, &cs.d_cluster);
  HIP_CHECK(hipStreamSynchronize(in.st));
  phase("lists merged");
  cs.iso_n = iso_m.n;
  std::swap(cs.iso_idx, iso_m.idx);
  std::swap(cs.iso_goff, iso_m.goff);
}

void ClusterStage::run(const StageInput &in, double w, int fast)
{
  uint64_t mg = 0;
  for (uint32_t g = 0; g < in.jr.n_groups && g + 1 < in.gstart_host.size(); ++g) mg = std::max<uint64_t>(mg, in.gstart_host[g + 1] - in.gstart_host[g]);
  for (auto &l : lanes) l->cb.max_group_bound = mg;
  if (lanes_apply(in, fast))
  {
    in.timed("mask_and_cluster_lanes", [&] { group_lanes(*this, in, w, fast); });
    return;
  }
  SvcStage svc_stage(*this, in.device, in.st, true, in.jr.n_pairs + 2ull * in.jr.n_groups + 4096, cb().max_group_bound, {in.st});
  in.timed("remove_isolated", [&] {
    const uint32_t *drop = in.own_groups.empty() ? nullptr : upload_drop(plan_owned(in), 1, d_drop, in.st);
    remove_isolated_all(in.jr.pairs, in.jr.gof, in.jr.gstart, in.jr.n_groups, in.jr.n_pairs, w, list, cb(), in.st, drop);
  });
  iso_n = list.n;
  snapshot_list(list, iso_idx, nullptr, iso_goff, in.st);
  if (!fast) svc_stage.finish();
  in.timed(fast ? "fast_cluster" : "ahc_cluster", [&] { cluster_list(in.jr.pairs, list, w, fast, d_cluster, cb(), ab, in.st); });
  svc_stage.finish();
}

void ClusterStage::sort_forms(uint64_t out[3]) const
{
  out[0] = out[1] = out[2] = 0;
  for (const auto &l : lanes)
    for (int k = 0; k < 2; ++k) out[k] += l->cb.se.sorts[k];
}

void ClusterStage::debug_sort(int device, hipStream_t st, uint32_t *key, uint32_t *idx, const uint32_t *gof, const uint64_t *goff, uint32_t ng, uint64_t n, uint64_t max_group)
{
  SvcStage svc_stage(*this, device, st, true, n + 2ull * ng + 4096, max_group, {st});
  std_sort_groups(key, idx, gof, goff, ng, n, cb().se, st);
  svc_stage.finish();
}
```

### breakid_amd/csrc/sortemu.h

```cpp
#pragma once
#include "bk_common.h"
#include <vector>
#include <atomic>

struct SortService
{
  DevBuf ctl, slots[2], seq[2], jobs, dbg, pos[2];
  uint32_t pos_cap[2] = {0, 0};
  uint32_t cap[2] = {0, 0};
  hipStream_t st[2] = {nullptr, nullptr}, quit_stream = nullptr, st_copy = nullptr;
  uint32_t *quit_host = nullptr;
  uint32_t *quit_dev = nullptr;
  uint32_t cap32 = 0;
  uint32_t quit_word = 0, starts = 0;
  size_t wide_lds = 0;
  bool running = false;
  std::atomic<uint32_t> next_slot{0};
  uint32_t stats[8] = {};
  void start(uint64_t n_bound, uint64_t max_group, hipStream_t after);
  bool narrow_running(double seconds) const;
  void stop();
  uint32_t new_slot() { return next_slot.fetch_add(1u); }
  ~SortService();
  SortService() = default;
  SortService(const SortService &) = delete;
  SortService &operator=(const SortService &) = delete;
};

struct SortEmuBufs
{
  SortService *svc = nullptr;
  uint32_t svc_slot = 0xFFFFFFFFu, svc_epoch = 0;
  DevBuf heap_scratch, scratch32, scratch32b, rk_a, rk_b, chk_key0, chk_cnt, chk_bad;
  std::vector<uint32_t> *heavy = nullptr;
  bool heavy_all = false;
  DevBuf tj_ctl, tj_jobs, tj_slots[2], tj_seq[2], tj_pos[2], tj_heavy, tj_trace;
  uint32_t tj_cap[2] = {0, 0}, tj_epoch = 0;
  bool tj_ready = false;
  uint64_t sorts[2] = {0, 0};
  SortEmuBufs() = default;
  SortEmuBufs(const SortEmuBufs &) = delete;
  SortEmuBufs &operator=(const SortEmuBufs &) = delete;
};

void std_sort_groups(uint32_t *key, uint32_t *idx, const uint32_t *gof, const uint64_t *goff, uint32_t ng, uint64_t n, SortEmuBufs &b, hipStream_t st);
```

### breakid_amd/csrc/sortemu.hip

```cpp
#include "bk_common.h"
#include "sortemu.h"
#include <vector>
#include <mutex>
#include <algorithm>
#include <cstdio>
#include <chrono>
#include <thread>
#include <cstdlib>

namespace
{
typedef __attribute__((address_space(1))) uint32_t gu32_t;
__device__ __forceinline__ void st_through(uint32_t *p, uint32_t v) { __hip_atomic_store((gu32_t *) p, v, __ATOMIC_RELAXED, __HIP_MEMORY_SCOPE_AGENT); }
constexpr uint32_t FIN_MAX = 2048;
constexpr uint32_t HEAP_BIG_MIN = 4096;

typedef unsigned long long hent;
__device__ __forceinline__ uint32_t hkey(hent e) { return (uint32_t) (e >> 32); }

struct E64
{
  typedef hent T;
  static __device__ __forceinline__ uint32_t key(T e) { return (uint32_t) (e >> 32); }
};
// ... 802 lines not shown
  if (x >= n)
  {
    atomicAdd(&bad[0], 1u);
    atomicMin(&bad[2], p);
    return;
  }
  if (atomicAdd(&cnt[x], 1u) != 0u)
  {
    atomicAdd(&bad[1], 1u);
    atomicMin(&bad[3], p);
  }
}
__global__ __launch_bounds__(256) void k_chk_keys(const uint32_t *__restrict__ key, const uint32_t *__restrict__ idx, const uint32_t *__restrict__ key0, uint32_t n, uint32_t *__restrict__ bad)
{
  const uint32_t p = blockIdx.x * blockDim.x + threadIdx.x;
  if (p >= n) return;
  const uint32_t x = idx[p];
  if (x < n && key0[x] != key[p])
  {
    atomicAdd(&bad[4], 1u);
    atomicMin(&bad[5], p);
  }
}
static void sort_check(const char *phase, const uint32_t *key, const uint32_t *idx, const uint32_t *key0, uint32_t n, const uint64_t *goff, uint32_t ng, hipStream_t st, SortEmuBufs &b)
{
  uint32_t *c = b.chk_cnt.as<uint32_t>(n), *bd = b.chk_bad.as<uint32_t>(8);
  const uint32_t init[8] = {0, 0, 0xFFFFFFFFu, 0xFFFFFFFFu, 0, 0xFFFFFFFFu, 0, 0};
  HIP_CHECK(hipDeviceSynchronize());
  HIP_CHECK(hipMemset(c, 0, (size_t) n * 4));
  HIP_CHECK(hipMemcpy(bd, init, 32, hipMemcpyHostToDevice));
  hipLaunchKernelGGL(k_chk_count, dim3(cdiv(n, 256)), dim3(256), 0, st, idx, n, c, bd);
  hipLaunchKernelGGL(k_chk_keys, dim3(cdiv(n, 256)), dim3(256), 0, st, key, idx, key0, n, bd);
  uint32_t h[8];
  HIP_CHECK(hipMemcpyAsync(h, bd, 32, hipMemcpyDeviceToHost, st));
  HIP_CHECK(hipStreamSynchronize(st));
  if (h[0] || h[1] || h[4])
  {
    std::vector<uint64_t> go((size_t) ng + 1);
    HIP_CHECK(hipMemcpy(go.data(), goff, ((size_t) ng + 1) * 8, hipMemcpyDeviceToHost));
    auto grp = [&](uint32_t p) { return p == 0xFFFFFFFFu ? -1 : (int) (std::upper_bound(go.begin(), go.end(), (uint64_t) p) - go.begin()) - 1; };
    fprintf(stderr, "[sortemu] CHECK FAILED %s: %u payloads out of range (first at %u), %u duplicated payloads (first at position %u, group %d), %u elements whose key is not their own (first at %u, group %d); n=%u\n",
            phase, h[0], h[2], h[1], h[3], grp(h[3]), h[4], h[5], grp(h[5]), n);
  }
}

struct WideLds
{
  size_t dyn_lds;
  uint32_t cap32;
};
static WideLds wide_lds_split(const void *kernel)
{
  hipFuncAttributes fa;
  HIP_CHECK(hipFuncGetAttributes(&fa, kernel));
  WideLds w;
  w.dyn_lds = (size_t) ((160u * 1024u - (uint32_t) fa.sharedSizeBytes) & ~15u);
  w.cap32 = (uint32_t) (w.dyn_lds / 4 - 3);
  if ((w.cap32 & 1u) == 0) --w.cap32;
  if ((w.cap32 & 1u) == 0 || 2ull * (w.cap32 + 1ull) <= HEAP_RANKED_MAX)
    throw bk_error(BK_ERR_HIP, "sort: " + std::to_string(fa.sharedSizeBytes) + " bytes of static LDS leave too little for the ranked heaps");
  return w;
}

static SvcParams svc_params(SortService &S)
{
  SvcParams P;
  uint32_t *ctl = S.ctl.get<uint32_t>();
  for (int k = 0; k < 2; ++k)
  {
    P.q[k].head = ctl + 64 * k;
    P.q[k].tail = ctl + 64 * k + 32;
    P.q[k].slots = S.slots[k].get<SvcTask>();
    P.q[k].seq = S.seq[k].get<uint32_t>();
    P.q[k].mask = S.cap[k] - 1;
    P.q[k].release = 1u;
  }
  P.error = ctl + 128;
  P.stats = ctl + 160;
  P.jobs = S.jobs.get<SvcJob>();
  P.quit_d = ctl + 192;
  P.host = S.quit_dev;
  P.cap32 = S.cap32;
  P.quit_word = S.quit_word;
  P.dbg = S.dbg.get<uint32_t>();
  for (int k = 0; k < 2; ++k)
  {
    P.pos[k] = S.pos[k].get<uint32_t>();
    P.pos_cap[k] = S.pos_cap[k];
  }
  P.timeout_ticks = SVC_TIMEOUT_TICKS;
  return P;
}
void SortService::start(uint64_t n_bound, uint64_t max_group, hipStream_t after)
{
  if (running) return;
  quit_stream = after;
  int dev = 0, cus = 0;
  HIP_CHECK(hipGetDevice(&dev));
  HIP_CHECK(hipDeviceGetAttribute(&cus, hipDeviceAttributeMultiprocessorCount, dev));
  const int n_wide = std::min(1024, std::max(4, cus / 4));
  const int n_narrow = std::max(8, 2 * (cus - n_wide));
  if (!quit_host)
  {
    HIP_CHECK(hipHostMalloc(reinterpret_cast<void **>(&quit_host), SVC_H_WORDS * 4, hipHostMallocMapped));
    HIP_CHECK(hipHostGetDevicePointer(reinterpret_cast<void **>(&quit_dev), quit_host, 0));
    for (int k = 0; k < 2; ++k) HIP_CHECK(hipStreamCreateWithFlags(&st[k], hipStreamNonBlocking));
    HIP_CHECK(hipStreamCreateWithFlags(&st_copy, hipStreamNonBlocking));
    const WideLds w = wide_lds_split(reinterpret_cast<const void *>(k_sort_service<true>));
    wide_lds = w.dyn_lds;
    cap32 = w.cap32;
    HIP_CHECK(hipFuncSetAttribute(reinterpret_cast<const void *>(k_sort_service<true>), hipFuncAttributeMaxDynamicSharedMemorySize, (int) wide_lds));
    HIP_CHECK(hipFuncSetAttribute(reinterpret_cast<const void *>(k_sort_service<false>), hipFuncAttributeMaxDynamicSharedMemorySize, (int) SVC_NARROW_LDS));
  }
  auto pow2 = [](uint64_t v) {
    uint32_t c = 1024;
    while (c < v && c < (1u << 30)) c <<= 1;
    return c;
  };
  cap[0] = pow2(n_bound / HEAP_BIG_MIN + 4096);
  cap[1] = pow2(n_bound / 16 + 4096);
  (void) ctl.as<uint32_t>(256);
  for (int k = 0; k < 2; ++k)
  {
    (void) slots[k].as<SvcTask>(cap[k]);
    (void) seq[k].as<uint32_t>(cap[k]);
  }
  (void) jobs.as<SvcJob>(SVC_MAX_JOBS);
  pos_cap[0] = (uint32_t) std::max<uint64_t>(max_group, SVC_WIDE_MIN) + 64;
  pos_cap[1] = SVC_WIDE_MIN + 64;
  (void) pos[0].as<uint32_t>(2ull * pos_cap[0] * (uint64_t) n_wide);
  (void) pos[1].as<uint32_t>(2ull * pos_cap[1] * (uint64_t) n_narrow);
  if (bk_debug("svc"))
  {
    (void) dbg.as<uint32_t>(12 * 8192 + 48);
    HIP_CHECK(hipMemsetAsync(dbg.p, 0, (12 * 8192 + 48) * 4, after));
  }
  __atomic_store_n(quit_host, 0u, __ATOMIC_SEQ_CST);
  quit_word = 0xC0DE0000u | (++starts & 0xFFFFu);
  for (uint32_t k = 1; k < SVC_H_WORDS; ++k) quit_host[k] = 0u;
  next_slot = 0;
  const SvcParams P = svc_params(*this);
  hipLaunchKernelGGL(k_svc_reset, dim3(cdiv(std::max(cap[0], cap[1]), 256)), dim3(256), 0, after, P);
  HIP_CHECK(hipStreamSynchronize(after));
  DeferredFrees::begin();
  running = true;
  hipLaunchKernelGGL(k_sort_service<true>, dim3(n_wide), dim3(1024), wide_lds, st[0], P);
  HIP_CHECK(hipGetLastError());
  {
    const auto t0 = std::chrono::steady_clock::now();
    volatile uint32_t *started = quit_host + SVC_H_STARTED;
    for (;;)
    {
      int have = 0;
      for (int k = 0; k < n_wide; ++k) have += started[k] != 0u;
      if (have == n_wide) break;
      if (std::chrono::duration<double>(std::chrono::steady_clock::now() - t0).count() > 0.25) break;
    }
  }
  hipLaunchKernelGGL(k_sort_service<false>, dim3(n_narrow), dim3(256), SVC_NARROW_LDS, st[1], P);
  HIP_CHECK(hipGetLastError());
}
bool SortService::narrow_running(double seconds) const
{
  const auto t0 = std::chrono::steady_clock::now();
  volatile const uint32_t *flag = quit_host + SVC_H_NARROW;
  while (*flag == 0u)
    if (std::chrono::duration<double>(std::chrono::steady_clock::now() - t0).count() > seconds) return false;
  return true;
}
void SortService::stop()
{
  if (!running) return;
  running = false;
  __atomic_store_n(quit_host, quit_word, __ATOMIC_SEQ_CST);
  (void) hipMemcpyAsync(ctl.get<uint32_t>() + 192, quit_host, 4, hipMemcpyHostToDevice, st_copy);
  hipLaunchKernelGGL(k_svc_quit, dim3(1), dim3(1), 0, quit_stream, ctl.get<uint32_t>() + 192, quit_word);
  HIP_CHECK(hipStreamSynchronize(st[0]));
  HIP_CHECK(hipStreamSynchronize(st[1]));
  uint32_t h[40] = {};
  HIP_CHECK(hipMemcpy(h, ctl.get<uint32_t>() + 128, sizeof h, hipMemcpyDeviceToHost));
  for (int k = 0; k < 8; ++k) stats[k] = h[32 + k];
  DeferredFrees::end();
  if (bk_debug("svc"))
  {
    uint32_t c[128] = {};
    SvcJob j0 = {};
    HIP_CHECK(hipMemcpy(c, ctl.get<uint32_t>(), sizeof c, hipMemcpyDeviceToHost));
    HIP_CHECK(hipMemcpy(&j0, jobs.get<SvcJob>(), sizeof j0, hipMemcpyDeviceToHost));
    if (dbg.p)
    {
      std::vector<uint32_t> d(12 * 8192 + 48);
      HIP_CHECK(hipMemcpy(d.data(), dbg.p, d.size() * 4, hipMemcpyDeviceToHost));
      {
        const uint32_t *ph = d.data() + 12 * 8192 + 32;
        const double lv = ph[7] ? (double) ph[7] : 1.0;
        fprintf(stderr, "[svc]   wide partition nodes: %u levels; per level: count pass %.2f us, place pass %.2f us, swaps + drain %.2f us, cut, release, pushes and the next pivot %.2f us\n", ph[7], ph[0] * 1e-2 / lv,
                ph[1] * 1e-2 / lv, ph[2] * 1e-2 / lv, ph[3] * 1e-2 / lv);
      }
      for (int kind = 0; kind < 2; ++kind)
      {
        fprintf(stderr, "[svc]   %s tasks by size (2^k ..):", kind ? "narrow heap" : "finisher");
        for (int k = 4; k < 13; ++k) fprintf(stderr, " %d:%u", k, d[12 * 8192 + 16 * kind + k]);
        fprintf(stderr, "\n");
      }
      for (int kind = 0; kind < 2; ++kind)
      {
        const uint32_t nw = kind == 0 ? stats[2] : stats[3];
        double sum[8] = {};
        uint32_t longest = 0;
        for (uint32_t w = 0; w < nw && w < 4096; ++w)
        {
          const uint32_t *a = d.data() + 4 * 8192 + 8 * (w + 4096 * kind);
          for (int k = 0; k < 7; ++k) sum[k] += a[k];
          longest = std::max(longest, a[7]);
        }
        fprintf(stderr, "[svc]   %s workgroups (%u): waiting %.2f ms; partition nodes %.0f in %.2f ms, finisher %.0f in %.2f ms, heaps %.0f in %.2f ms (sums over the workgroups); longest task %.3f ms\n", kind ? "narrow" : "wide", nw,
                sum[0] * 1e-5, sum[4], sum[1] * 1e-5, sum[5], sum[2] * 1e-5, sum[6], sum[3] * 1e-5, longest * 1e-5);
        std::map<uint32_t, int> hist;
        const uint32_t n = kind == 0 ? stats[2] : stats[3];
        for (uint32_t w = 0; w < n && w < 4096; ++w) hist[d[4 * (w + 4096 * kind)]]++;
        fprintf(stderr, "[svc]   %s workgroups by last state (1 polling, 5 took a task, 9 left):", kind ? "narrow" : "wide");
        for (auto &kv : hist) fprintf(stderr, " %u:%d", kv.first, kv.second);
        fprintf(stderr, "; first ones (state, polls, time of the last poll in 10 ns, how it left 6 error 7 quit 8 timeout):");
        for (uint32_t w = 0; w < 6 && w < n; ++w) fprintf(stderr, " [%u %u %u %u]", d[4 * (w + 4096 * kind)], d[4 * (w + 4096 * kind) + 1], d[4 * (w + 4096 * kind) + 2], d[4 * (w + 4096 * kind) + 3]);
        fprintf(stderr, "\n");
      }
    }
    uint32_t sq[4] = {};
    HIP_CHECK(hipMemcpy(sq, seq[1].get<uint32_t>(), sizeof sq, hipMemcpyDeviceToHost));
    fprintf(stderr, "[svc] tasks %u wide / %u narrow; workgroups started %u / %u, left on their own %u / %u, odd quit words read %u; error %u; wide queue head %u tail %u, narrow queue head %u tail %u (seq %u %u %u %u); job 0: remaining %u done %u heaps %u (longest %u)\n",
            stats[0], stats[1], stats[2], stats[3], stats[4], stats[5], stats[6], h[0], c[0], c[32], c[64], c[96], sq[0], sq[1], sq[2], sq[3], j0.remaining, j0.done, j0.n_heap, j0.max_heap);
  }
  if (h[0]) throw bk_error(h[0] & 2u ? BK_ERR_LIMIT : BK_ERR_HIP, "sort service: task error " + std::to_string(h[0]) + " (2 = ring overflow, 4 = a job timed out, 8 = a cut outside its segment, 16 = a task in the wrong queue, 32 = a node beyond the position lists, 64 = the finisher); first failing task: code " + std::to_string(h[8]) + ", " + std::to_string(h[9]) + " " + std::to_string(h[10]) + " " + std::to_string(h[11]));
}
SortService::~SortService()
{
  if (running)
  {
    running = false;
    if (quit_host && st_copy)
    {
      __atomic_store_n(quit_host, quit_word, __ATOMIC_SEQ_CST);
      (void) hipMemcpyAsync(ctl.get<uint32_t>() + 192, quit_host, 4, hipMemcpyHostToDevice, st_copy);
    }
    if (quit_stream) hipLaunchKernelGGL(k_svc_quit, dim3(1), dim3(1), 0, quit_stream, ctl.get<uint32_t>() + 192, quit_word);
    for (int k = 0; k < 2; ++k)
      if (st[k]) (void) hipStreamSynchronize(st[k]);
    DeferredFrees::end();
  }
  for (int k = 0; k < 2; ++k)
    if (st[k]) (void) hipStreamDestroy(st[k]);
  if (st_copy) (void) hipStreamDestroy(st_copy);
  if (quit_host) (void) hipHostFree(quit_host);
}

static void window_sorts(uint32_t *key, uint32_t *idx, const uint32_t *gof, uint32_t n, hipStream_t st);

static void std_sort_groups_svc(uint32_t *key, uint32_t *idx, const uint32_t *gof, const uint64_t *goff, uint32_t ng, uint32_t n, SortEmuBufs &b, hipStream_t st)
{
  SortService &S = *b.svc;
  if (b.svc_slot == 0xFFFFFFFFu)
  {
    b.svc_slot = S.new_slot();
    if (b.svc_slot >= SVC_MAX_JOBS) throw bk_error(BK_ERR_LIMIT, "sort service: more than 64 callers");
  }
  SvcJob d = {};
  d.key = key;
  d.idx = idx;
  d.hscratch = b.heap_scratch.as<hent>((uint64_t) n + HEAP_PAD);
  d.scratch32 = b.scratch32.as<uint32_t>((uint64_t) n + HEAP_PAD);
  d.scratch32b = b.scratch32b.as<uint32_t>((uint64_t) n + HEAP_PAD);
  d.rka = b.rk_a.as<unsigned long long>((uint64_t) n + HEAP_PAD);
  d.rkb = b.rk_b.as<unsigned long long>((uint64_t) n + HEAP_PAD);
  d.epoch = (b.svc_epoch++ % 0xFFFFFu) + 1u;
  const SvcParams P = svc_params(S);
  hipLaunchKernelGGL(k_svc_submit, dim3(1), dim3(256), 0, st, P, d, b.svc_slot, goff, ng);
  HIP_CHECK(hipGetLastError());
  {
    volatile const uint32_t *done = S.quit_host + SVC_H_DONE + b.svc_slot, *err = S.quit_host + SVC_H_ERROR;
    const auto t0 = std::chrono::steady_clock::now();
    for (uint32_t spins = 0; *done != d.epoch; ++spins)
    {
      if (*err != 0u)
        throw bk_error(BK_ERR_HIP, "sort service: a task failed (error " + std::to_string(*err) + "; first failing task: code " + std::to_string(err[1]) + ", " + std::to_string(err[2]) + " " + std::to_string(err[3]) + " " + std::to_string(err[4]) + ")");
      if ((spins & 1023u) == 1023u)
      {
        if (std::chrono::duration<double>(std::chrono::steady_clock::now() - t0).count() > 20.0) throw bk_error(BK_ERR_HIP, "sort service: a job did not finish");
        std::this_thread::yield();
      }
      else
        __builtin_ia32_pause();
    }
  }
  if (bk_debug("svc"))
  {
    SvcJob j;
    HIP_CHECK(hipMemcpy(&j, S.jobs.get<SvcJob>() + b.svc_slot, sizeof j, hipMemcpyDeviceToHost));
    fprintf(stderr, "[svc] slot %u sort %u: %u elements in %u groups; partitions and finisher done after %.3f ms, job after %.3f ms; %u elements in heaps, the longest %u, the heap that ended last %u elements in %.3f ms\n", b.svc_slot,
            b.svc_epoch, n, ng, (double) (j.t_parts - j.t_submit) * 1e-5, (double) (j.t_done - j.t_submit) * 1e-5, j.n_heap, j.max_heap, (uint32_t) j.last_heap, (double) (j.last_heap >> 32) * 1e-5);
  }
  window_sorts(key, idx, gof, n, st);
}

static void std_sort_groups_tasks(uint32_t *key, uint32_t *idx, const uint32_t *gof, const uint64_t *goff, uint32_t ng, uint32_t n, SortEmuBufs &b, hipStream_t st, const uint32_t *key0)
{
  static size_t dyn_lds = 0;
  static uint32_t cap32 = 0;
  static std::once_flag once;
  std::call_once(once, [] {
    const WideLds w = wide_lds_split(reinterpret_cast<const void *>(k_sort_job));
    dyn_lds = w.dyn_lds;
    cap32 = w.cap32;
    if (dyn_lds < SJ_TEAMS * SJ_TEAM_LDS) throw bk_error(BK_ERR_HIP, "k_sort_job: the narrow teams do not fit the LDS");
    HIP_CHECK(hipFuncSetAttribute(reinterpret_cast<const void *>(k_sort_job), hipFuncAttributeMaxDynamicSharedMemorySize, (int) dyn_lds));
  });
  std::vector<uint64_t> go((size_t) ng + 1);
  HIP_CHECK(hipMemcpyAsync(go.data(), goff, go.size() * 8, hipMemcpyDeviceToHost, st));
  HIP_CHECK(hipStreamSynchronize(st));
  uint64_t max_group = 0;
  for (uint32_t g = 0; g < ng; ++g) max_group = std::max<uint64_t>(max_group, go[g + 1] - go[g]);
  const uint32_t n_wide = std::min<uint32_t>(SJ_MAX_WIDE, std::max<uint32_t>(1, cdiv(n, 1u << 16)));
  const uint32_t n_narrow = std::min<uint32_t>(SJ_MAX_NARROW, std::max<uint32_t>(1, cdiv(n, 1u << 16)));
  SjParams S = {};
  SvcParams &P = S.P;
  {
    auto pow2 = [](uint64_t v) {
      uint32_t c = 1024;
      while (c < v && c < (1u << 30)) c <<= 1;
      return c;
    };
    const uint32_t want[2] = {pow2((uint64_t) n / HEAP_BIG_MIN + 4096), pow2((uint64_t) n / 16 + 4096)};
    for (int k = 0; k < 2; ++k)
      if (want[k] > b.tj_cap[k])
      {
        b.tj_cap[k] = want[k];
        b.tj_ready = false;
      }
    uint32_t *ctl = b.tj_ctl.as<uint32_t>(SJ_C_WORDS);
    for (int k = 0; k < 2; ++k)
    {
      P.q[k].head = ctl + 64 * k;
      P.q[k].tail = ctl + 64 * k + 32;
      P.q[k].slots = b.tj_slots[k].as<SvcTask>(b.tj_cap[k]);
      P.q[k].seq = b.tj_seq[k].as<uint32_t>(b.tj_cap[k]);
      P.q[k].mask = b.tj_cap[k] - 1;
      P.q[k].release = 1u;
    }
    P.error = ctl + SJ_C_ERROR;
    P.stats = ctl + SJ_C_STATS;
    P.quit_d = ctl + SJ_C_QUIT;
    P.host = ctl + SJ_C_HOST;
    P.jobs = b.tj_jobs.as<SvcJob>(SVC_MAX_JOBS);
    P.cap32 = cap32;
    P.quit_word = 0u;
    P.timeout_ticks = SJ_TIMEOUT_TICKS;
    P.pos_cap[0] = (uint32_t) std::max<uint64_t>(max_group, SVC_WIDE_MIN) + 64;
    P.pos_cap[1] = SVC_WIDE_MIN + 64;
    P.pos[0] = b.tj_pos[0].as<uint32_t>(2ull * P.pos_cap[0] * n_wide);
    P.pos[1] = b.tj_pos[1].as<uint32_t>(2ull * P.pos_cap[1] * n_narrow * SJ_TEAMS);
    P.dbg = nullptr;
    S.n_wide = n_wide;
    S.live = ctl + SJ_C_LIVE;
    S.gof = gof;
    S.heavy_min = b.heavy_all ? FIN_MAX : HEAP_RANKED_MIN;
    if (b.heavy)
    {
      S.heavy = b.tj_heavy.as<uint32_t>(ng);
      HIP_CHECK(hipMemsetAsync(S.heavy, 0, (size_t) ng * 4, st));
    }
  }
  static const bool dbg = bk_debug("svc");
  if (dbg) S.trace = b.tj_trace.as<unsigned long long>(8);
  if (!b.tj_ready)
  {
    HIP_CHECK(hipMemsetAsync(b.tj_ctl.p, 0, SJ_C_WORDS * 4, st));
    hipLaunchKernelGGL(k_svc_reset, dim3(cdiv(std::max(b.tj_cap[0], b.tj_cap[1]), 256)), dim3(256), 0, st, P);
    b.tj_ready = true;
  }
  SvcJob d = {};
  d.key = key;
  d.idx = idx;
  d.hscratch = b.heap_scratch.as<hent>((uint64_t) n + HEAP_PAD);
  d.scratch32 = b.scratch32.as<uint32_t>((uint64_t) n + HEAP_PAD);
  d.scratch32b = b.scratch32b.as<uint32_t>((uint64_t) n + HEAP_PAD);
  d.rka = b.rk_a.as<unsigned long long>((uint64_t) n + HEAP_PAD);
  d.rkb = b.rk_b.as<unsigned long long>((uint64_t) n + HEAP_PAD);
  d.epoch = (b.tj_epoch++ % 0xFFFFFu) + 1u;
  const SvcJobLds J = {d.key, d.idx, nullptr, nullptr, d.hscratch, d.scratch32, d.scratch32b, d.rka, d.rkb, P.jobs, d.epoch << 8};
  hipLaunchKernelGGL(k_sort_job_submit, dim3(1), dim3(256), 0, st, S, d, goff, ng);
  hipLaunchKernelGGL(k_sort_job, dim3(n_wide + n_narrow), dim3(1024), dyn_lds, st, S, J);
  HIP_CHECK(hipGetLastError());
  ++b.sorts[1];
  if (key0) sort_check("after the task dispatch", key, idx, key0, n, goff, ng, st, b);
  window_sorts(key, idx, gof, n, st);
  uint32_t h[16] = {};
  HIP_CHECK(hipMemcpyAsync(h, P.error, 12 * 4, hipMemcpyDeviceToHost, st));
  std::vector<uint32_t> hv;
  if (S.heavy)
  {
    hv.resize(ng);
    HIP_CHECK(hipMemcpyAsync(hv.data(), S.heavy, (size_t) ng * 4, hipMemcpyDeviceToHost, st));
  }
  unsigned long long tr[8] = {};
  if (S.trace) HIP_CHECK(hipMemcpyAsync(tr, S.trace, 5 * 8, hipMemcpyDeviceToHost, st));
  SvcJob j = {};
  HIP_CHECK(hipMemcpyAsync(&j, P.jobs, sizeof j, hipMemcpyDeviceToHost, st));
  HIP_CHECK(hipStreamSynchronize(st));
  if (h[0] || j.remaining != 0u)
  {
    b.tj_ready = false;
    throw bk_error(h[0] & 2u ? BK_ERR_LIMIT : BK_ERR_HIP, "sort task dispatch: task error " + std::to_string(h[0]) + " (2 = ring overflow, 4 = no progress for 1 s, 8 = a cut outside its segment, 16 = a task in the wrong queue, 32 = a node beyond the position lists, 64 = the finisher), " + std::to_string(j.remaining) + " elements not final; first failing task: code " + std::to_string(h[8]) + ", " + std::to_string(h[9]) + " " + std::to_string(h[10]) + " " + std::to_string(h[11]));
  }
  if (S.heavy)
  {
    if (b.heavy->size() < ng) b.heavy->resize(ng, 0u);
    for (uint32_t g = 0; g < ng; ++g) (*b.heavy)[g] = std::max((*b.heavy)[g], hv[g]);
  }
  if (S.trace)
  {
    const double t0 = (double) tr[0];
    const uint32_t hm = (uint32_t) (tr[1] >> 40);
    const unsigned long long hs = tr[1] & 0xFFFFFFFFFFull, base = tr[0] & ~0xFFFFFFFFFFull;
    unsigned long long hstart = base | hs;
    if (hstart < tr[0]) hstart += 1ull << 40;
    fprintf(stderr, "[svc] task dispatch %u: %u elements in %u groups on %u wide + %u narrow workgroups; longest heap %u elements started %.3f ms after the dispatch and took %.3f ms; partitions and finisher done after %.3f ms, job after %.3f ms; %u elements in heaps, the longest %u\n",
            d.epoch, n, ng, n_wide, n_narrow, hm, hm ? ((double) hstart - t0) * 1e-5 : 0.0, hm ? (double) (tr[2] & 0xFFFFFFFFFFull) * 1e-5 : 0.0, tr[3] ? ((double) tr[3] - t0) * 1e-5 : 0.0, ((double) tr[4] - t0) * 1e-5, j.n_heap, j.max_heap);
  }
}

void std_sort_groups(uint32_t *key, uint32_t *idx, const uint32_t *gof, const uint64_t *goff, uint32_t ng, uint64_t n64, SortEmuBufs &b, hipStream_t st)
{
  if (n64 == 0 || ng == 0) return;
  if (n64 > 0x7FFFFFF0ull) throw bk_error(BK_ERR_LIMIT, "std_sort_groups: more than 2^31 pairs");
  const uint32_t n = (uint32_t) n64;
  if (b.svc && b.svc->running)
  {
    ++b.sorts[0];
    std_sort_groups_svc(key, idx, gof, goff, ng, n, b, st);
    return;
  }
  static const bool chk = bk_debug("sortcheck");
  DevBuf &chk_key0 = b.chk_key0;
  uint32_t *key0 = nullptr;
  if (chk)
  {
    key0 = chk_key0.as<uint32_t>(n);
    std::vector<uint32_t> hk(n), hx(n), k0(n);
    HIP_CHECK(hipStreamSynchronize(st));
    HIP_CHECK(hipMemcpy(hk.data(), key, (size_t) n * 4, hipMemcpyDeviceToHost));
    HIP_CHECK(hipMemcpy(hx.data(), idx, (size_t) n * 4, hipMemcpyDeviceToHost));
    for (uint32_t i = 0; i < n; ++i)
      if (hx[i] < n) k0[hx[i]] = hk[i];
    HIP_CHECK(hipMemcpy(key0, k0.data(), (size_t) n * 4, hipMemcpyHostToDevice));
    sort_check("at entry", key, idx, key0, n, goff, ng, st, b);
  }
  if (const char *dump = getenv("BK_DEBUG_SORT_DUMP"))
  {
    static int call = 0;
    if (call < 5)
    {
      std::vector<uint64_t> go((size_t) ng + 1);
      std::vector<uint32_t> kk(n);
      HIP_CHECK(hipStreamSynchronize(st));
      HIP_CHECK(hipMemcpy(go.data(), goff, ((size_t) ng + 1) * 8, hipMemcpyDeviceToHost));
      HIP_CHECK(hipMemcpy(kk.data(), key, (size_t) n * 4, hipMemcpyDeviceToHost));
      char name[512];
      snprintf(name, sizeof name, "%s.%d.keys.u32", dump, call);
      if (FILE *f = fopen(name, "wb"))
      {
        fwrite(kk.data(), 4, kk.size(), f);
        fclose(f);
      }
      snprintf(name, sizeof name, "%s.%d.goff.u64", dump, call);
      if (FILE *f = fopen(name, "wb"))
      {
        fwrite(go.data(), 8, go.size(), f);
        fclose(f);
      }
    }
    ++call;
  }
  std_sort_groups_tasks(key, idx, gof, goff, ng, n, b, st, chk ? key0 : nullptr);
}
static void window_sorts(uint32_t *key, uint32_t *idx, const uint32_t *gof, uint32_t n, hipStream_t st)
{
  hipLaunchKernelGGL(k_se_window_sort, dim3(cdiv(n, 256)), dim3(256), 0, st, key, idx, gof, n, 0u);
  if (n > 16) hipLaunchKernelGGL(k_se_window_sort, dim3(cdiv(n - 16, 256)), dim3(256), 0, st, key, idx, gof, n, 16u);
}
```

Measured before the change: 11690.

## Cut host syncs and launches in clustering: fuse kernels, pass group bound, skip merge

Fuses key gather with iota and the multi-array permutation gathers into one kernel, folds the group-offset and start-mark kernels into neighbouring kernels, and swaps buffers instead of copying back. It passes a known maximum group size into the sort so the device-to-host copy of offsets and the sync can be skipped. It also replaces the full merge of masked lanes with an offsets-only merge plus per-lane subset gathers, and lets the old list be handed over instead of snapshotted. The aim is fewer launches, syncs and device copies, at the cost of more buffer juggling and reliance on the supplied group bound being correct.

```diff
diff --git a/breakid_amd/csrc/api.hip b/breakid_amd/csrc/api.hip
--- a/breakid_amd/csrc/api.hip
+++ b/breakid_amd/csrc/api.hip
@@ -2576,6 +2576,9 @@
     if (n) HIP_CHECK(hipMemcpy(dgof.as<uint32_t>(n + 1), gof.data(), n * 4, hipMemcpyHostToDevice));
     HIP_CHECK(hipMemcpy(dgoff.as<uint64_t>((uint64_t) n_groups + 1), group_off, goff_bytes, hipMemcpyHostToDevice));
     const bk_pair *pairs = dp.as<bk_pair>(n + 1);
+    uint64_t largest = 0;
+    for (uint32_t g = 0; g < n_groups; ++g) largest = std::max<uint64_t>(largest, group_off[g + 1] - group_off[g]);
+    ctx->stage.cb().max_group_bound = largest;
     if (mode == 1)
       remove_isolated_all(pairs, dgof.get<uint32_t>(), dgoff.get<uint64_t>(), n_groups, n, w, L, ctx->stage.cb(), ctx->st);
     else
diff --git a/breakid_amd/csrc/cluster.h b/breakid_amd/csrc/cluster.h
--- a/breakid_amd/csrc/cluster.h
+++ b/breakid_amd/csrc/cluster.h
@@ -14,6 +14,7 @@
   DevBuf idx;
   DevBuf gof;
   DevBuf goff;
+  std::vector<uint64_t> goff_host;
   uint64_t total(hipStream_t st) const;
 };
 
@@ -22,7 +23,9 @@
   std::vector<uint32_t> heavy_x, heavy_y;
   bool observe = false;
   uint64_t max_group_bound = 0;
-  DevBuf key, perm, tmp, cnt, off, off2, idx2, gof2, goff2, jump, mark, apos, kid, kprev2, k1, k2, pk, knum, clfull, small, scan_tmp;
+  PairList *snap = nullptr;
+  DevBuf key, perm, tmp, cnt, off, off2, idx2, gof2, goff2, jump, mark, apos, kid, kprev2, k2alt, k1, k2, pk, knum, clfull, scan_tmp;
+  uint32_t host_words[2] = {0, 0};
   SortEmuBufs se;
   prims::RadixBufs radix;
 };
@@ -32,8 +35,10 @@
 void remove_isolated_begin(const bk_pair *pairs, const uint32_t *gof0, const uint64_t *gstart, uint32_t ng, uint64_t n, double w, PairList &L, ClusterBufs &b, hipStream_t st,
                            const uint32_t *drop_group = nullptr, const uint64_t *gstart_host = nullptr, const uint8_t *keep_host = nullptr);
 void remove_isolated_end(const bk_pair *pairs, PairList &L, ClusterBufs &b, hipStream_t st);
-void list_subset_ranges(const PairList &src, const uint64_t *src_goff_host, const uint8_t *keep_host, PairList &dst, hipStream_t st);
+void list_subset_of_lists(const PairList *const *lists, int K, const uint64_t *goff_host, const uint8_t *keep_host, PairList &dst, hipStream_t st);
+void merged_group_offsets(const PairList *const *lists, int K, DevBuf &goff_out, hipStream_t st);
 void drop_small_groups(PairList &L, ClusterBufs &b, hipStream_t st);
 void fast_cluster_all(const bk_pair *pairs, PairList &L, double w, DevBuf &cluster_out, ClusterBufs &b, hipStream_t st);
+constexpr int LISTS_MAX = 26;
 void merge_lists_many(const PairList *const *lists, const uint32_t *const *cls, int K, PairList &out, DevBuf *cl_out, hipStream_t st);
 void debug_mask_list(const bk_pair *pairs, PairList &L, long dist, ClusterBufs &b, hipStream_t st);
diff --git a/breakid_amd/csrc/cluster.hip b/breakid_amd/csrc/cluster.hip
--- a/breakid_amd/csrc/cluster.hip
+++ b/breakid_amd/csrc/cluster.hip
@@ -17,10 +17,23 @@
   uint64_t p = (uint64_t) blockIdx.x * blockDim.x + threadIdx.x;
   if (p < n) key[p] = use_y ? pairs[idx[p]].y : pairs[idx[p]].x;
 }
-__global__ __launch_bounds__(256) void k_gather_u32(const uint32_t *__restrict__ src, const uint32_t *__restrict__ perm, uint64_t n, uint32_t *__restrict__ dst)
-{
-  uint64_t p = (uint64_t) blockIdx.x * blockDim.x + threadIdx.x;
-  if (p < n) dst[p] = src[perm[p]];
+__global__ __launch_bounds__(256) void k_key_iota(const bk_pair *__restrict__ pairs, const uint32_t *__restrict__ idx, uint64_t n, int use_y, uint32_t *__restrict__ key,
+                                                  uint32_t *__restrict__ perm)
+{
+  uint64_t p = (uint64_t) blockIdx.x * blockDim.x + threadIdx.x;
+  if (p >= n) return;
+  key[p] = use_y ? pairs[idx[p]].y : pairs[idx[p]].x;
+  perm[p] = (uint32_t) p;
+}
+__global__ __launch_bounds__(256) void k_gather_perm(const uint32_t *__restrict__ perm, uint64_t n, const uint32_t *__restrict__ a0, const uint32_t *__restrict__ a1,
+                                                     const uint32_t *__restrict__ a2, uint32_t *__restrict__ o0, uint32_t *__restrict__ o1, uint32_t *__restrict__ o2)
+{
+  uint64_t p = (uint64_t) blockIdx.x * blockDim.x + threadIdx.x;
+  if (p >= n) return;
+  const uint32_t q = perm[p];
+  o0[p] = a0[q];
+  if (a1) o1[p] = a1[q];
+  if (a2) o2[p] = a2[q];
 }
 
 __device__ __forceinline__ long absdiff(uint32_t a, uint32_t b)
@@ -56,10 +69,18 @@
   cnt[p] = c;
 }
 
+__device__ __forceinline__ void new_goff(uint64_t g, const uint32_t *__restrict__ off, const uint64_t *__restrict__ goff, uint32_t ng, uint64_t n, uint64_t *__restrict__ ogoff)
+{
+  if (g > ng) return;
+  const uint64_t s = g < ng ? goff[g] : n;
+  ogoff[g] = off[s];
+}
 __global__ __launch_bounds__(256) void k_expand(const uint32_t *__restrict__ cnt, const uint32_t *__restrict__ off, const uint32_t *__restrict__ idx,
-                                                const uint32_t *__restrict__ gof, uint64_t n, uint32_t *__restrict__ oidx, uint32_t *__restrict__ ogof)
-{
-  uint64_t p = (uint64_t) blockIdx.x * blockDim.x + threadIdx.x;
+                                                const uint32_t *__restrict__ gof, uint64_t n, uint32_t *__restrict__ oidx, uint32_t *__restrict__ ogof,
+                                                const uint64_t *__restrict__ goff, uint32_t ng, uint64_t *__restrict__ ogoff)
+{
+  uint64_t p = (uint64_t) blockIdx.x * blockDim.x + threadIdx.x;
+  new_goff(p, off, goff, ng, n, ogoff);
   if (p >= n) return;
   uint32_t c = cnt[p], o = off[p];
   for (uint32_t k = 0; k < c; ++k)
@@ -68,21 +89,16 @@
     ogof[o + k] = gof[p];
   }
 }
-__global__ void k_new_goff(const uint32_t *__restrict__ off, const uint64_t *__restrict__ goff, uint32_t ng, uint64_t n, uint64_t *__restrict__ ogoff)
-{
-  uint32_t g = blockIdx.x * blockDim.x + threadIdx.x;
-  if (g > ng) return;
-  uint64_t s = g < ng ? goff[g] : n;
-  ogoff[g] = off[s];
-}
 
 __global__ __launch_bounds__(256) void k_fast_next(const uint32_t *__restrict__ key, const uint32_t *__restrict__ gof, const uint64_t *__restrict__ goff, uint64_t n, double w,
-                                                   uint32_t *__restrict__ nxt)
+                                                   uint32_t *__restrict__ nxt, uint32_t *__restrict__ mark)
 {
   uint64_t p = (uint64_t) blockIdx.x * blockDim.x + threadIdx.x;
   if (p >= n) return;
   uint32_t g = gof[p];
   uint64_t ge = goff[g + 1];
+  mark[p] = goff[g] == p ? 1u : 0u;
+  if (p == n - 1) mark[n] = 0u;
   if (p + 1 >= ge)
   {
     nxt[p] = END;
@@ -97,12 +113,6 @@
   }
   if (lo > ge - 1) lo = ge - 1;
   nxt[p] = (uint32_t) lo;
-}
-__global__ void k_mark_starts(const uint64_t *__restrict__ goff, uint32_t ng, uint32_t *__restrict__ mark)
-{
-  uint32_t g = blockIdx.x * blockDim.x + threadIdx.x;
-  if (g >= ng) return;
-  if (goff[g + 1] > goff[g]) mark[goff[g]] = 1;
 }
 __global__ __launch_bounds__(FW_TILE) void k_fw_exit(const uint32_t *__restrict__ nxt, uint64_t n, uint32_t *__restrict__ exitp)
 {
@@ -167,10 +177,12 @@
   if (p < n && mark[p]) apos[ascan[p]] = (uint32_t) p;
 }
 __global__ __launch_bounds__(256) void k_fast_keep(const uint32_t *__restrict__ mark, const uint32_t *__restrict__ ascan, const uint32_t *__restrict__ apos,
-                                                   const uint32_t *__restrict__ nxt, uint64_t n, uint32_t *__restrict__ keep, uint32_t *__restrict__ kid)
-{
-  uint64_t p = (uint64_t) blockIdx.x * blockDim.x + threadIdx.x;
-  if (p >= n) return;
+                                                   const uint32_t *__restrict__ nxt, uint64_t n, uint32_t *__restrict__ keep, uint32_t *__restrict__ kid,
+                                                   uint32_t *__restrict__ n_anchors)
+{
+  uint64_t p = (uint64_t) blockIdx.x * blockDim.x + threadIdx.x;
+  if (p >= n) return;
+  if (p == 0) *n_anchors = ascan[n];
   uint32_t ord = ascan[p] + mark[p] - 1;
   uint32_t a = apos[ord];
   uint32_t e = nxt[a];
@@ -179,9 +191,11 @@
 }
 __global__ __launch_bounds__(256) void k_compact3(const uint32_t *__restrict__ keep, const uint32_t *__restrict__ off, uint64_t n, const uint32_t *__restrict__ a0,
                                                   const uint32_t *__restrict__ a1, const uint32_t *__restrict__ a2, const uint32_t *__restrict__ a3, uint32_t *__restrict__ o0,
-                                                  uint32_t *__restrict__ o1, uint32_t *__restrict__ o2, uint32_t *__restrict__ o3)
-{
-  uint64_t p = (uint64_t) blockIdx.x * blockDim.x + threadIdx.x;
+                                                  uint32_t *__restrict__ o1, uint32_t *__restrict__ o2, uint32_t *__restrict__ o3,
+                                                  const uint64_t *__restrict__ goff, uint32_t ng, uint64_t *__restrict__ ogoff)
+{
+  uint64_t p = (uint64_t) blockIdx.x * blockDim.x + threadIdx.x;
+  new_goff(p, off, goff, ng, n, ogoff);
   if (p >= n || !keep[p]) return;
   uint32_t o = off[p];
   o0[o] = a0[p];
@@ -241,10 +255,12 @@
   uint64_t p = (uint64_t) blockIdx.x * blockDim.x + threadIdx.x;
   if (p < n) cl[p] = keep[p] ? knum[uid[p]] : 0u;
 }
-__global__ void k_group_small(const uint64_t *__restrict__ goff, uint32_t ng, uint32_t *__restrict__ small)
-{
-  uint32_t g = blockIdx.x * blockDim.x + threadIdx.x;
-  if (g < ng) small[g] = (goff[g + 1] - goff[g]) < 2 ? 1u : 0u;
+__global__ __launch_bounds__(256) void k_keep_large(const uint32_t *__restrict__ gof, const uint64_t *__restrict__ goff, uint64_t n, uint32_t *__restrict__ keep)
+{
+  uint64_t p = (uint64_t) blockIdx.x * blockDim.x + threadIdx.x;
+  if (p >= n) return;
+  const uint32_t g = gof[p];
+  keep[p] = (goff[g + 1] - goff[g]) < 2 ? 0u : 1u;
 }
 __global__ __launch_bounds__(256) void k_drop_small(const uint32_t *__restrict__ gof, const uint32_t *__restrict__ small, uint64_t n, uint32_t *__restrict__ keep)
 {
@@ -263,24 +279,39 @@
 }
 
 static inline unsigned nb(uint64_t n) { return cdiv(n ? n : 1, 256); }
+static const uint32_t *scan_total(const uint32_t *dev, int words, ClusterBufs &b, hipStream_t st)
+{
+  uint32_t *h = b.host_words;
+  HIP_CHECK(hipMemcpyAsync(h, dev, (size_t) words * 4, hipMemcpyDeviceToHost, st));
+  HIP_CHECK(hipStreamSynchronize(st));
+  return h;
+}
 static void filter_groups(PairList &L, const uint32_t *drop, ClusterBufs &b, hipStream_t st);
 
-static void sort_list(const bk_pair *pairs, PairList &L, int use_y, uint32_t **extra, int n_extra, ClusterBufs &b, hipStream_t st)
+static void sort_list(const bk_pair *pairs, PairList &L, int use_y, DevBuf *k1, DevBuf *k2, ClusterBufs &b, hipStream_t st)
 {
   if (L.n == 0) return;
   uint32_t *key = b.key.as<uint32_t>(L.n), *perm = b.perm.as<uint32_t>(L.n);
-  hipLaunchKernelGGL(k_gather_key, dim3(nb(L.n)), dim3(256), 0, st, pairs, L.idx.get<uint32_t>(), L.n, use_y, key);
-  hipLaunchKernelGGL(k_iota, dim3(nb(L.n)), dim3(256), 0, st, perm, L.n);
+  hipLaunchKernelGGL(k_key_iota, dim3(nb(L.n)), dim3(256), 0, st, pairs, L.idx.get<uint32_t>(), L.n, use_y, key, perm);
   b.se.heavy = b.observe ? (use_y ? &b.heavy_y : &b.heavy_x) : nullptr;
-  std_sort_groups(key, perm, L.gof.get<uint32_t>(), L.goff.get<uint64_t>(), L.ng, L.n, b.se, st);
+  std_sort_groups(key, perm, L.gof.get<uint32_t>(), L.goff.get<uint64_t>(), L.ng, L.n, b.se, st, b.max_group_bound ? b.max_group_bound + 2 : 0);
   b.se.heavy = nullptr;
-  uint32_t *tmp = b.tmp.as<uint32_t>(L.n);
-  auto apply = [&](uint32_t *arr) {
-    hipLaunchKernelGGL(k_gather_u32, dim3(nb(L.n)), dim3(256), 0, st, arr, perm, L.n, tmp);
-    HIP_CHECK(hipMemcpyAsync(arr, tmp, L.n * 4, hipMemcpyDeviceToDevice, st));
-  };
-  apply(L.idx.get<uint32_t>());
-  for (int k = 0; k < n_extra; ++k) apply(extra[k]);
+  uint32_t *oidx = b.idx2.as<uint32_t>(L.n + 1);
+  uint32_t *o1 = k1 ? b.kprev2.as<uint32_t>(L.n + 1) : nullptr, *o2 = k2 ? b.k2alt.as<uint32_t>(L.n + 1) : nullptr;
+  hipLaunchKernelGGL(k_gather_perm, dim3(nb(L.n)), dim3(256), 0, st, perm, L.n, L.idx.get<uint32_t>(), k1 ? k1->get<uint32_t>() : nullptr, k2 ? k2->get<uint32_t>() : nullptr, oidx,
+                     o1, o2);
+  std::swap(L.idx, b.idx2);
+  if (k1) std::swap(*k1, b.kprev2);
+  if (k2) std::swap(*k2, b.k2alt);
+}
+
+static void hand_over_old_list(ClusterBufs &b)
+{
+  if (!b.snap) return;
+  std::swap(b.snap->idx, b.idx2);
+  std::swap(b.snap->gof, b.gof2);
+  std::swap(b.snap->goff, b.goff2);
+  b.snap = nullptr;
 }
 
 static void mask_list(const bk_pair *pairs, PairList &L, long dist, ClusterBufs &b, hipStream_t st)
@@ -290,13 +321,11 @@
   hipLaunchKernelGGL(k_mask_count, dim3(nb(L.n)), dim3(256), 0, st, pairs, L.idx.get<uint32_t>(), L.gof.get<uint32_t>(), L.goff.get<uint64_t>(), L.n, dist, cnt);
   uint32_t *off = b.off.as<uint32_t>(L.n + 1);
   prims::exclusive_scan<uint32_t>(cnt, off, L.n, b.scan_tmp, st);
-  uint32_t total = 0;
-  HIP_CHECK(hipMemcpyAsync(&total, off + L.n, 4, hipMemcpyDeviceToHost, st));
-  HIP_CHECK(hipStreamSynchronize(st));
+  const uint32_t total = scan_total(off + L.n, 1, b, st)[0];
   uint32_t *oidx = b.idx2.as<uint32_t>((uint64_t) total + 1), *ogof = b.gof2.as<uint32_t>((uint64_t) total + 1);
   uint64_t *ogoff = b.goff2.as<uint64_t>((uint64_t) L.ng + 1);
-  hipLaunchKernelGGL(k_expand, dim3(nb(L.n)), dim3(256), 0, st, cnt, off, L.idx.get<uint32_t>(), L.gof.get<uint32_t>(), L.n, oidx, ogof);
-  hipLaunchKernelGGL(k_new_goff, dim3(cdiv(L.ng + 1, 256)), dim3(256), 0, st, off, L.goff.get<uint64_t>(), L.ng, L.n, ogoff);
+  hipLaunchKernelGGL(k_expand, dim3(nb(std::max<uint64_t>(L.n, (uint64_t) L.ng + 1))), dim3(256), 0, st, cnt, off, L.idx.get<uint32_t>(), L.gof.get<uint32_t>(), L.n, oidx, ogof,
+                     L.goff.get<uint64_t>(), L.ng, ogoff);
   std::swap(L.idx, b.idx2);
   std::swap(L.gof, b.gof2);
   std::swap(L.goff, b.goff2);
@@ -313,7 +342,7 @@
 void remove_isolated_end(const bk_pair *pairs, PairList &L, ClusterBufs &b, hipStream_t st)
 {
   if (L.n == 0 || L.ng == 0) return;
-  sort_list(pairs, L, 0, nullptr, 0, b, st);
+  sort_list(pairs, L, 0, nullptr, nullptr, b, st);
 }
 
 namespace
@@ -333,47 +362,16 @@
   gof[p] = lo;
 }
 }
-namespace
-{
-__global__ __launch_bounds__(256) void k_subset_of_list(const uint32_t *__restrict__ src_idx, const uint64_t *__restrict__ src_goff, const uint64_t *__restrict__ goff, uint32_t ng,
-                                                        uint64_t n_list, uint32_t *__restrict__ idx, uint32_t *__restrict__ gof)
-{
-  const uint64_t p = (uint64_t) blockIdx.x * blockDim.x + threadIdx.x;
-  if (p >= n_list) return;
-  uint32_t lo = 0, hi = ng;
-  while (hi - lo > 1)
-  {
-    const uint32_t m = (lo + hi) >> 1;
-    if (goff[m] <= p) lo = m; else hi = m;
-  }
-  idx[p] = src_idx[src_goff[lo] + (p - goff[lo])];
-  gof[p] = lo;
-}
-}
-void list_subset_ranges(const PairList &src, const uint64_t *src_goff_host, const uint8_t *keep_host, PairList &dst, hipStream_t st)
-{
-  const uint32_t ng = src.ng;
-  std::vector<uint64_t> goff((size_t) ng + 1, 0);
-  for (uint32_t g = 0; g < ng; ++g) goff[g + 1] = goff[g] + (keep_host[g] ? src_goff_host[g + 1] - src_goff_host[g] : 0);
-  dst.n = goff[ng];
-  dst.ng = ng;
-  uint32_t *idx = dst.idx.as<uint32_t>(dst.n + 1), *gof = dst.gof.as<uint32_t>(dst.n + 1);
-  uint64_t *dgoff = dst.goff.as<uint64_t>((uint64_t) ng + 1);
-  HIP_CHECK(hipMemcpyAsync(dgoff, goff.data(), ((size_t) ng + 1) * 8, hipMemcpyHostToDevice, st));
-  HIP_CHECK(hipStreamSynchronize(st));
-  if (dst.n) hipLaunchKernelGGL(k_subset_of_list, dim3(nb(dst.n)), dim3(256), 0, st, src.idx.get<uint32_t>(), src.goff.get<uint64_t>(), dgoff, ng, dst.n, idx, gof);
-}
-
 void list_of_groups(const uint64_t *gstart_dev, const uint64_t *gstart_host, const uint8_t *keep_host, uint32_t ng, PairList &L, hipStream_t st)
 {
-  std::vector<uint64_t> goff((size_t) ng + 1, 0);
+  std::vector<uint64_t> &goff = L.goff_host;
+  goff.assign((size_t) ng + 1, 0);
   for (uint32_t g = 0; g < ng; ++g) goff[g + 1] = goff[g] + (keep_host[g] ? gstart_host[g + 1] - gstart_host[g] : 0);
   L.n = goff[ng];
   L.ng = ng;
   uint32_t *idx = L.idx.as<uint32_t>(L.n + 1), *gof = L.gof.as<uint32_t>(L.n + 1);
   uint64_t *dgoff = L.goff.as<uint64_t>((uint64_t) ng + 1);
   HIP_CHECK(hipMemcpyAsync(dgoff, goff.data(), ((size_t) ng + 1) * 8, hipMemcpyHostToDevice, st));
-  HIP_CHECK(hipStreamSynchronize(st));
   if (L.n) hipLaunchKernelGGL(k_subset_list, dim3(nb(L.n)), dim3(256), 0, st, gstart_dev, dgoff, ng, L.n, idx, gof);
 }
 
@@ -408,23 +406,21 @@
   }
   if (L.n == 0) return;
   const long dist = (long) w;
-  sort_list(pairs, L, 0, nullptr, 0, b, st);
+  sort_list(pairs, L, 0, nullptr, nullptr, b, st);
   mask_list(pairs, L, dist, b, st);
-  sort_list(pairs, L, 1, nullptr, 0, b, st);
+  sort_list(pairs, L, 1, nullptr, nullptr, b, st);
   mask_list(pairs, L, dist, b, st);
 }
 
-static void fast_pass(const bk_pair *pairs, PairList &L, int use_y, double w, DevBuf &k_prev, DevBuf &k_new, ClusterBufs &b, hipStream_t st)
-{
-  if (L.n == 0) return;
+static uint32_t fast_pass(const bk_pair *pairs, PairList &L, int use_y, double w, DevBuf &k_prev, DevBuf &k_new, ClusterBufs &b, hipStream_t st)
+{
+  if (L.n == 0) return 0;
   const uint64_t n = L.n;
   uint32_t *key = b.key.as<uint32_t>(n);
   hipLaunchKernelGGL(k_gather_key, dim3(nb(n)), dim3(256), 0, st, pairs, L.idx.get<uint32_t>(), n, use_y, key);
   uint32_t *jump = b.jump.as<uint32_t>(n * 2ull);
-  hipLaunchKernelGGL(k_fast_next, dim3(nb(n)), dim3(256), 0, st, key, L.gof.get<uint32_t>(), L.goff.get<uint64_t>(), n, w, jump);
   uint32_t *mark = b.mark.as<uint32_t>(n + 1);
-  HIP_CHECK(hipMemsetAsync(mark, 0, (n + 1) * 4, st));
-  hipLaunchKernelGGL(k_mark_starts, dim3(cdiv(L.ng, 256)), dim3(256), 0, st, L.goff.get<uint64_t>(), L.ng, mark);
+  hipLaunchKernelGGL(k_fast_next, dim3(nb(n)), dim3(256), 0, st, key, L.gof.get<uint32_t>(), L.goff.get<uint64_t>(), n, w, jump, mark);
   {
     uint32_t *exitp = jump + n;
     const unsigned tiles = (unsigned) cdiv(n, FW_TILE);
@@ -437,82 +433,79 @@
   uint32_t *apos = b.apos.as<uint32_t>(n + 1);
   hipLaunchKernelGGL(k_anchor_pos, dim3(nb(n)), dim3(256), 0, st, mark, ascan, n, apos);
   uint32_t *keep = b.cnt.as<uint32_t>(n + 1), *kid = b.kid.as<uint32_t>(n + 1);
-  hipLaunchKernelGGL(k_fast_keep, dim3(nb(n)), dim3(256), 0, st, mark, ascan, apos, jump, n, keep, kid);
-  uint32_t *off = b.off2.as<uint32_t>(n + 1);
+  uint32_t *off = b.off2.as<uint32_t>(n + 2);
+  hipLaunchKernelGGL(k_fast_keep, dim3(nb(n)), dim3(256), 0, st, mark, ascan, apos, jump, n, keep, kid, off + n + 1);
   prims::exclusive_scan<uint32_t>(keep, off, n, b.scan_tmp, st);
-  uint32_t total = 0;
-  HIP_CHECK(hipMemcpyAsync(&total, off + n, 4, hipMemcpyDeviceToHost, st));
-  HIP_CHECK(hipStreamSynchronize(st));
+  const uint32_t *both = scan_total(off + n, 2, b, st);
+  const uint32_t total = both[0], anchors = both[1];
   uint32_t *oidx = b.idx2.as<uint32_t>((uint64_t) total + 1), *ogof = b.gof2.as<uint32_t>((uint64_t) total + 1);
   uint32_t *okn = k_new.as<uint32_t>((uint64_t) total + 1);
   uint32_t *okp = k_prev.p ? b.kprev2.as<uint32_t>((uint64_t) total + 1) : nullptr;
   uint64_t *ogoff = b.goff2.as<uint64_t>((uint64_t) L.ng + 1);
-  hipLaunchKernelGGL(k_compact3, dim3(nb(n)), dim3(256), 0, st, keep, off, n, L.idx.get<uint32_t>(), L.gof.get<uint32_t>(), kid, k_prev.get<uint32_t>(), oidx, ogof, okn, okp);
-  hipLaunchKernelGGL(k_new_goff, dim3(cdiv(L.ng + 1, 256)), dim3(256), 0, st, off, L.goff.get<uint64_t>(), L.ng, n, ogoff);
+  hipLaunchKernelGGL(k_compact3, dim3(nb(std::max<uint64_t>(n, (uint64_t) L.ng + 1))), dim3(256), 0, st, keep, off, n, L.idx.get<uint32_t>(), L.gof.get<uint32_t>(), kid,
+                     k_prev.get<uint32_t>(), oidx, ogof, okn, okp, L.goff.get<uint64_t>(), L.ng, ogoff);
   std::swap(L.idx, b.idx2);
   std::swap(L.gof, b.gof2);
   std::swap(L.goff, b.goff2);
   if (k_prev.p) std::swap(k_prev, b.kprev2);
   L.n = total;
+  hand_over_old_list(b);
+  return anchors;
 }
 
 static void filter_groups(PairList &L, const uint32_t *drop, ClusterBufs &b, hipStream_t st)
 {
   if (L.n == 0) return;
   uint32_t *keep = b.cnt.as<uint32_t>(L.n + 1), *off = b.off.as<uint32_t>(L.n + 1);
-  hipLaunchKernelGGL(k_drop_small, dim3(nb(L.n)), dim3(256), 0, st, L.gof.get<uint32_t>(), drop, L.n, keep);
+  if (drop)
+    hipLaunchKernelGGL(k_drop_small, dim3(nb(L.n)), dim3(256), 0, st, L.gof.get<uint32_t>(), drop, L.n, keep);
+  else
+    hipLaunchKernelGGL(k_keep_large, dim3(nb(L.n)), dim3(256), 0, st, L.gof.get<uint32_t>(), L.goff.get<uint64_t>(), L.n, keep);
   prims::exclusive_scan<uint32_t>(keep, off, L.n, b.scan_tmp, st);
-  uint32_t total = 0;
-  HIP_CHECK(hipMemcpyAsync(&total, off + L.n, 4, hipMemcpyDeviceToHost, st));
-  HIP_CHECK(hipStreamSynchronize(st));
+  const uint32_t total = scan_total(off + L.n, 1, b, st)[0];
   if (total != L.n)
   {
     uint32_t *oidx = b.idx2.as<uint32_t>((uint64_t) total + 1), *ogof = b.gof2.as<uint32_t>((uint64_t) total + 1);
     uint64_t *ogoff = b.goff2.as<uint64_t>((uint64_t) L.ng + 1);
-    hipLaunchKernelGGL(k_compact3, dim3(nb(L.n)), dim3(256), 0, st, keep, off, L.n, L.idx.get<uint32_t>(), L.gof.get<uint32_t>(), (const uint32_t *) nullptr,
-                       (const uint32_t *) nullptr, oidx, ogof, (uint32_t *) nullptr, (uint32_t *) nullptr);
-    hipLaunchKernelGGL(k_new_goff, dim3(cdiv(L.ng + 1, 256)), dim3(256), 0, st, off, L.goff.get<uint64_t>(), L.ng, L.n, ogoff);
+    hipLaunchKernelGGL(k_compact3, dim3(nb(std::max<uint64_t>(L.n, (uint64_t) L.ng + 1))), dim3(256), 0, st, keep, off, L.n, L.idx.get<uint32_t>(), L.gof.get<uint32_t>(),
+                       (const uint32_t *) nullptr, (const uint32_t *) nullptr, oidx, ogof, (uint32_t *) nullptr, (uint32_t *) nullptr, L.goff.get<uint64_t>(), L.ng, ogoff);
     std::swap(L.idx, b.idx2);
     std::swap(L.gof, b.gof2);
     std::swap(L.goff, b.goff2);
     L.n = total;
+    hand_over_old_list(b);
   }
 }
 
 void drop_small_groups(PairList &L, ClusterBufs &b, hipStream_t st)
 {
   if (L.n == 0) return;
-  uint32_t *small = b.small.as<uint32_t>((uint64_t) L.ng + 1);
-  hipLaunchKernelGGL(k_group_small, dim3(cdiv(L.ng, 256)), dim3(256), 0, st, L.goff.get<uint64_t>(), L.ng, small);
-  filter_groups(L, small, b, st);
+  filter_groups(L, nullptr, b, st);
 }
 
 void fast_cluster_all(const bk_pair *pairs, PairList &L, double w, DevBuf &cluster_out, ClusterBufs &b, hipStream_t st)
 {
   drop_small_groups(L, b, st);
   DevBuf none;
-  const uint64_t n_first = L.n;
-  fast_pass(pairs, L, 0, w, none, b.k1, b, st);
-  {
-    uint32_t *extra[1] = {b.k1.get<uint32_t>()};
-    sort_list(pairs, L, 1, extra, L.n ? 1 : 0, b, st);
-  }
-  fast_pass(pairs, L, 1, w, b.k1, b.k2, b, st);
-  {
-    uint32_t *extra[2] = {b.k1.get<uint32_t>(), b.k2.get<uint32_t>()};
-    sort_list(pairs, L, 0, extra, L.n ? 2 : 0, b, st);
-  }
+  const uint32_t anchors1 = fast_pass(pairs, L, 0, w, none, b.k1, b, st);
+  sort_list(pairs, L, 1, &b.k1, nullptr, b, st);
+  const uint32_t anchors2 = fast_pass(pairs, L, 1, w, b.k1, b.k2, b, st);
+  sort_list(pairs, L, 0, &b.k1, &b.k2, b, st);
   const uint64_t n = L.n;
   uint32_t *cl = cluster_out.as<uint32_t>(n + 1);
   if (n == 0) return;
   uint64_t *pk = b.pk.as<uint64_t>(n);
   uint32_t *pv = b.perm.as<uint32_t>(n);
-  int kbits = 1;
-  while (kbits < 32 && (n_first >> kbits) != 0) ++kbits;
-  hipLaunchKernelGGL(k_pack_k, dim3(nb(n)), dim3(256), 0, st, b.k1.get<uint32_t>(), b.k2.get<uint32_t>(), n, kbits, pk, pv);
+  auto bits = [](uint32_t v) {
+    int k = 1;
+    while (k < 32 && (v >> k) != 0) ++k;
+    return k;
+  };
+  const int kbits1 = bits(anchors1), kbits2 = bits(anchors2);
+  hipLaunchKernelGGL(k_pack_k, dim3(nb(n)), dim3(256), 0, st, b.k1.get<uint32_t>(), b.k2.get<uint32_t>(), n, kbits1, pk, pv);
   uint64_t *ks;
   uint32_t *vs;
-  prims::radix_sort_pairs(pk, pv, n, 0, std::min(64, 2 * kbits), b.radix, st, &ks, &vs);
+  prims::radix_sort_pairs(pk, pv, n, 0, kbits1 + kbits2, b.radix, st, &ks, &vs);
   uint32_t *flag = b.cnt.as<uint32_t>(n + 1), *fscan = b.off.as<uint32_t>(n + 1);
   hipLaunchKernelGGL(k_run_flag, dim3(nb(n)), dim3(256), 0, st, ks, n, flag);
   prims::exclusive_scan<uint32_t>(flag, fscan, n, b.scan_tmp, st);
@@ -528,15 +521,12 @@
   hipLaunchKernelGGL(k_cluster_of, dim3(nb(n)), dim3(256), 0, st, uid, knum, keep, n, clfull);
   uint32_t *off = b.off.as<uint32_t>(n + 1);
   prims::exclusive_scan<uint32_t>(keep, off, n, b.scan_tmp, st);
-  uint32_t total = 0;
-  HIP_CHECK(hipMemcpyAsync(&total, off + n, 4, hipMemcpyDeviceToHost, st));
-  HIP_CHECK(hipStreamSynchronize(st));
+  const uint32_t total = scan_total(off + n, 1, b, st)[0];
   uint32_t *oidx = b.idx2.as<uint32_t>((uint64_t) total + 1), *ogof = b.gof2.as<uint32_t>((uint64_t) total + 1);
   uint64_t *ogoff = b.goff2.as<uint64_t>((uint64_t) L.ng + 1);
   cl = cluster_out.as<uint32_t>((uint64_t) total + 1);
-  hipLaunchKernelGGL(k_compact3, dim3(nb(n)), dim3(256), 0, st, keep, off, n, L.idx.get<uint32_t>(), L.gof.get<uint32_t>(), clfull, (const uint32_t *) nullptr, oidx, ogof, cl,
-                     (uint32_t *) nullptr);
-  hipLaunchKernelGGL(k_new_goff, dim3(cdiv(L.ng + 1, 256)), dim3(256), 0, st, off, L.goff.get<uint64_t>(), L.ng, n, ogoff);
+  hipLaunchKernelGGL(k_compact3, dim3(nb(std::max<uint64_t>(n, (uint64_t) L.ng + 1))), dim3(256), 0, st, keep, off, n, L.idx.get<uint32_t>(), L.gof.get<uint32_t>(), clfull,
+                     (const uint32_t *) nullptr, oidx, ogof, cl, (uint32_t *) nullptr, L.goff.get<uint64_t>(), L.ng, ogoff);
   std::swap(L.idx, b.idx2);
   std::swap(L.gof, b.gof2);
   std::swap(L.goff, b.goff2);
@@ -547,21 +537,71 @@
 
 namespace
 {
-__global__ __launch_bounds__(256) void k_merge_goff(const uint64_t *__restrict__ b, uint32_t ng, uint64_t *__restrict__ out)
+struct ListSet
+{
+  const uint32_t *idx[LISTS_MAX], *gof[LISTS_MAX], *cl[LISTS_MAX];
+  const uint64_t *goff[LISTS_MAX];
+  uint64_t start[LISTS_MAX + 1];
+  int K;
+};
+ListSet list_set(const PairList *const *lists, const uint32_t *const *cls, int K)
+{
+  if (K < 1 || K > LISTS_MAX) throw bk_error(BK_ERR_ARG, "more lists than a merge takes");
+  ListSet M = {};
+  M.K = K;
+  for (int l = 0; l < K; ++l)
+  {
+    M.idx[l] = lists[l]->idx.get<uint32_t>();
+    M.gof[l] = lists[l]->gof.get<uint32_t>();
+    M.goff[l] = lists[l]->goff.get<uint64_t>();
+    M.cl[l] = cls ? cls[l] : nullptr;
+    M.start[l + 1] = M.start[l] + lists[l]->n;
+  }
+  return M;
+}
+__global__ __launch_bounds__(256) void k_merge_goff(const ListSet M, uint32_t ng, uint64_t *__restrict__ out)
 {
   uint32_t g = blockIdx.x * blockDim.x + threadIdx.x;
-  if (g <= ng) out[g] += b[g];
-}
-__global__ __launch_bounds__(256) void k_merge_copy(const uint32_t *__restrict__ idx, const uint32_t *__restrict__ gof, const uint32_t *__restrict__ cl, const uint64_t *__restrict__ goff,
-                                                    uint64_t n, const uint64_t *__restrict__ mgoff, uint32_t *__restrict__ oidx, uint32_t *__restrict__ ogof, uint32_t *__restrict__ ocl)
-{
-  uint64_t p = (uint64_t) blockIdx.x * blockDim.x + threadIdx.x;
-  if (p >= n) return;
-  const uint32_t g = gof[p];
-  const uint64_t d = mgoff[g] + (p - goff[g]);
-  oidx[d] = idx[p];
+  if (g > ng) return;
+  uint64_t s = 0;
+  for (int l = 0; l < M.K; ++l) s += M.goff[l][g];
+  out[g] = s;
+}
+__global__ __launch_bounds__(256) void k_merge_copy(const ListSet M, const uint64_t *__restrict__ mgoff, uint32_t *__restrict__ oidx, uint32_t *__restrict__ ogof,
+                                                    uint32_t *__restrict__ ocl)
+{
+  uint64_t p = (uint64_t) blockIdx.x * blockDim.x + threadIdx.x;
+  if (p >= M.start[M.K]) return;
+  int l = 0;
+  for (int k = 1; k < M.K; ++k)
+    if (p >= M.start[k]) l = k;
+  const uint64_t q = p - M.start[l];
+  const uint32_t g = M.gof[l][q];
+  const uint64_t d = mgoff[g] + (q - M.goff[l][g]);
+  oidx[d] = M.idx[l][q];
   ogof[d] = g;
-  if (cl) ocl[d] = cl[p];
+  if (ocl) ocl[d] = M.cl[l][q];
+}
+__global__ __launch_bounds__(256) void k_subset_of_lists(const ListSet M, const uint64_t *__restrict__ goff, uint32_t ng, uint64_t n_list, uint32_t *__restrict__ idx,
+                                                         uint32_t *__restrict__ gof)
+{
+  const uint64_t p = (uint64_t) blockIdx.x * blockDim.x + threadIdx.x;
+  if (p >= n_list) return;
+  uint32_t lo = 0, hi = ng;
+  while (hi - lo > 1)
+  {
+    const uint32_t m = (lo + hi) >> 1;
+    if (goff[m] <= p) lo = m; else hi = m;
+  }
+  const uint64_t i = p - goff[lo];
+  uint32_t v = 0;
+  for (int l = 0; l < M.K; ++l)
+  {
+    const uint64_t s = M.goff[l][lo];
+    if (i < M.goff[l][lo + 1] - s) v = M.idx[l][s + i];
+  }
+  idx[p] = v;
+  gof[p] = lo;
 }
 }
 
@@ -574,11 +614,28 @@
   uint32_t *oidx = out.idx.as<uint32_t>(out.n + 1), *ogof = out.gof.as<uint32_t>(out.n + 1);
   uint64_t *ogoff = out.goff.as<uint64_t>((uint64_t) ng + 1);
   uint32_t *ocl = cl_out ? cl_out->as<uint32_t>(out.n + 1) : nullptr;
-  HIP_CHECK(hipMemsetAsync(ogoff, 0, ((size_t) ng + 1) * 8, st));
-  for (int l = 0; l < K; ++l) hipLaunchKernelGGL(k_merge_goff, dim3(cdiv(ng + 1, 256)), dim3(256), 0, st, lists[l]->goff.get<uint64_t>(), ng, ogoff);
-  for (int l = 0; l < K; ++l)
-  {
-    const PairList &A = *lists[l];
-    if (A.n) hipLaunchKernelGGL(k_merge_copy, dim3(nb(A.n)), dim3(256), 0, st, A.idx.get<uint32_t>(), A.gof.get<uint32_t>(), cls ? cls[l] : nullptr, A.goff.get<uint64_t>(), A.n, ogoff, oidx, ogof, ocl);
-  }
-}
+  const ListSet M = list_set(lists, cl_out ? cls : nullptr, K);
+  hipLaunchKernelGGL(k_merge_goff, dim3(cdiv(ng + 1, 256)), dim3(256), 0, st, M, ng, ogoff);
+  if (out.n) hipLaunchKernelGGL(k_merge_copy, dim3(nb(out.n)), dim3(256), 0, st, M, ogoff, oidx, ogof, ocl);
+}
+
+void merged_group_offsets(const PairList *const *lists, int K, DevBuf &goff_out, hipStream_t st)
+{
+  const uint32_t ng = lists[0]->ng;
+  const ListSet M = list_set(lists, nullptr, K);
+  hipLaunchKernelGGL(k_merge_goff, dim3(cdiv(ng + 1, 256)), dim3(256), 0, st, M, ng, goff_out.as<uint64_t>((uint64_t) ng + 1));
+}
+
+void list_subset_of_lists(const PairList *const *lists, int K, const uint64_t *goff_host, const uint8_t *keep_host, PairList &dst, hipStream_t st)
+{
+  const uint32_t ng = lists[0]->ng;
+  std::vector<uint64_t> &goff = dst.goff_host;
+  goff.assign((size_t) ng + 1, 0);
+  for (uint32_t g = 0; g < ng; ++g) goff[g + 1] = goff[g] + (keep_host[g] ? goff_host[g + 1] - goff_host[g] : 0);
+  dst.n = goff[ng];
+  dst.ng = ng;
+  uint32_t *idx = dst.idx.as<uint32_t>(dst.n + 1), *gof = dst.gof.as<uint32_t>(dst.n + 1);
+  uint64_t *dgoff = dst.goff.as<uint64_t>((uint64_t) ng + 1);
+  HIP_CHECK(hipMemcpyAsync(dgoff, goff.data(), ((size_t) ng + 1) * 8, hipMemcpyHostToDevice, st));
+  if (dst.n) hipLaunchKernelGGL(k_subset_of_lists, dim3(nb(dst.n)), dim3(256), 0, st, list_set(lists, nullptr, K), dgoff, ng, dst.n, idx, gof);
+}
diff --git a/breakid_amd/csrc/lanes.h b/breakid_amd/csrc/lanes.h
--- a/breakid_amd/csrc/lanes.h
+++ b/breakid_amd/csrc/lanes.h
@@ -28,6 +28,7 @@
   {
     ClusterBufs cb;
     PairList list, iso;
+    PairList masked;
     DevBuf d_cluster;
     hipStream_t st = nullptr;
     ~Lane()
@@ -41,8 +42,8 @@
   PairList list;
   DevBuf d_cluster, iso_idx, iso_goff;
   uint64_t iso_n = 0;
-  PairList lane_mid, lane_iso_m;
-  DevBuf d_drop;
+  PairList lane_iso_m;
+  DevBuf d_drop, d_mid_goff;
 
   ClusterStage() { lanes.emplace_back(new Lane()); }
   void run(const StageInput &in, double w, int fast);
diff --git a/breakid_amd/csrc/lanes.hip b/breakid_amd/csrc/lanes.hip
--- a/breakid_amd/csrc/lanes.hip
+++ b/breakid_amd/csrc/lanes.hip
@@ -243,12 +243,33 @@
   if (L.n && ig) HIP_CHECK(hipMemcpyAsync(ig, L.gof.get<uint32_t>(), L.n * 4, hipMemcpyDeviceToDevice, st));
   if (L.ng) HIP_CHECK(hipMemcpyAsync(io, L.goff.get<uint64_t>(), ((uint64_t) L.ng + 1) * 8, hipMemcpyDeviceToDevice, st));
 }
-static void cluster_list(const bk_pair *pairs, PairList &L, double w, int fast, DevBuf &cl, ClusterBufs &cb, AhcBufs &ab, hipStream_t st)
-{
+static void cluster_list(const bk_pair *pairs, PairList &L, double w, int fast, DevBuf &cl, PairList &iso, bool iso_gof, ClusterBufs &cb, AhcBufs &ab, hipStream_t st)
+{
+  iso.n = L.n;
+  iso.ng = L.ng;
   if (fast)
-    fast_cluster_all(pairs, L, w, cl, cb, st);
+  {
+    cb.snap = &iso;
+    try
+    {
+      fast_cluster_all(pairs, L, w, cl, cb, st);
+    }
+    catch (...)
+    {
+      cb.snap = nullptr;
+      throw;
+    }
+    if (cb.snap)
+    {
+      cb.snap = nullptr;
+      snapshot_list(L, iso.idx, iso_gof ? &iso.gof : nullptr, iso.goff, st);
+    }
+  }
   else
+  {
+    snapshot_list(L, iso.idx, iso_gof ? &iso.gof : nullptr, iso.goff, st);
     ahc_cluster_all(pairs, L, w, cl, ab, cb, st);
+  }
 }
 
 using LanePlan = std::vector<int>;
@@ -442,11 +463,7 @@
     if (observe) cb.observe = false;
   };
   auto cluster_lane = [&](int l) {
-    PairList &L = lane(l).list, &iso = lane(l).iso;
-    iso.n = L.n;
-    iso.ng = L.ng;
-    snapshot_list(L, iso.idx, &iso.gof, iso.goff, lane_st(l));
-    cluster_list(pairs, L, w, fast, lane(l).d_cluster, lane(l).cb, cs.ab, lane_st(l));
+    cluster_list(pairs, lane(l).list, w, fast, lane(l).d_cluster, lane(l).iso, true, lane(l).cb, cs.ab, lane_st(l));
   };
   const auto tp0 = std::chrono::steady_clock::now();
   auto phase = [&](const char *what) {
@@ -462,10 +479,15 @@
   else
   {
     in_lanes([&](int l) { mask_lane(l, true); });
-    PairList &mid = cs.lane_mid;
-    merge_all(&ClusterStage::Lane::list, mid, nullptr);
+    std::vector<const PairList *> masked(K);
+    for (int l = 0; l < K; ++l)
+    {
+      std::swap(lane(l).list, lane(l).masked);
+      masked[l] = &lane(l).masked;
+    }
+    merged_group_offsets(masked.data(), K, cs.d_mid_goff, in.st);
     std::vector<uint64_t> goff_h((size_t) ng + 1);
-    HIP_CHECK(hipMemcpyAsync(goff_h.data(), mid.goff.get<uint64_t>(), ((size_t) ng + 1) * 8, hipMemcpyDeviceToHost, in.st));
+    HIP_CHECK(hipMemcpyAsync(goff_h.data(), cs.d_mid_goff.get<uint64_t>(), ((size_t) ng + 1) * 8, hipMemcpyDeviceToHost, in.st));
     HIP_CHECK(hipStreamSynchronize(in.st));
     std::vector<uint64_t> sizes(ng);
     std::vector<uint32_t> hx(ng, 0u), hy(ng, 0u);
@@ -478,7 +500,7 @@
       }
     upload_plan(plan_observed(sizes, hx, hy, K));
     in_lanes([&](int l) {
-      list_subset_ranges(mid, goff_h.data(), keep[l].data(), lane(l).list, lane_st(l));
+      list_subset_of_lists(masked.data(), K, goff_h.data(), keep[l].data(), lane(l).list, lane_st(l));
       cluster_lane(l);
     });
   }
@@ -512,9 +534,24 @@
     remove_isolated_all(in.jr.pairs, in.jr.gof, in.jr.gstart, in.jr.n_groups, in.jr.n_pairs, w, list, cb(), in.st, drop);
   });
   iso_n = list.n;
-  snapshot_list(list, iso_idx, nullptr, iso_goff, in.st);
   if (!fast) svc_stage.finish();
-  in.timed(fast ? "fast_cluster" : "ahc_cluster", [&] { cluster_list(in.jr.pairs, list, w, fast, d_cluster, cb(), ab, in.st); });
+  PairList &iso = lane_iso_m;
+  std::swap(iso.idx, iso_idx);
+  std::swap(iso.goff, iso_goff);
+  auto give_back = [&] {
+    std::swap(iso.idx, iso_idx);
+    std::swap(iso.goff, iso_goff);
+  };
+  try
+  {
+    in.timed(fast ? "fast_cluster" : "ahc_cluster", [&] { cluster_list(in.jr.pairs, list, w, fast, d_cluster, iso, false, cb(), ab, in.st); });
+  }
+  catch (...)
+  {
+    give_back();
+    throw;
+  }
+  give_back();
   svc_stage.finish();
 }
 
diff --git a/breakid_amd/csrc/sortemu.h b/breakid_amd/csrc/sortemu.h
--- a/breakid_amd/csrc/sortemu.h
+++ b/breakid_amd/csrc/sortemu.h
@@ -43,4 +43,4 @@
   SortEmuBufs &operator=(const SortEmuBufs &) = delete;
 };
 
-void std_sort_groups(uint32_t *key, uint32_t *idx, const uint32_t *gof, const uint64_t *goff, uint32_t ng, uint64_t n, SortEmuBufs &b, hipStream_t st);
+void std_sort_groups(uint32_t *key, uint32_t *idx, const uint32_t *gof, const uint64_t *goff, uint32_t ng, uint64_t n, SortEmuBufs &b, hipStream_t st, uint64_t max_group_bound = 0);
diff --git a/breakid_amd/csrc/sortemu.hip b/breakid_amd/csrc/sortemu.hip
--- a/breakid_amd/csrc/sortemu.hip
+++ b/breakid_amd/csrc/sortemu.hip
@@ -1128,7 +1128,8 @@
   window_sorts(key, idx, gof, n, st);
 }
 
-static void std_sort_groups_tasks(uint32_t *key, uint32_t *idx, const uint32_t *gof, const uint64_t *goff, uint32_t ng, uint32_t n, SortEmuBufs &b, hipStream_t st, const uint32_t *key0)
+static void std_sort_groups_tasks(uint32_t *key, uint32_t *idx, const uint32_t *gof, const uint64_t *goff, uint32_t ng, uint32_t n, SortEmuBufs &b, hipStream_t st, const uint32_t *key0,
+                                  uint64_t max_group_bound)
 {
   static size_t dyn_lds = 0;
   static uint32_t cap32 = 0;
@@ -1140,11 +1141,14 @@
     if (dyn_lds < SJ_TEAMS * SJ_TEAM_LDS) throw bk_error(BK_ERR_HIP, "k_sort_job: the narrow teams do not fit the LDS");
     HIP_CHECK(hipFuncSetAttribute(reinterpret_cast<const void *>(k_sort_job), hipFuncAttributeMaxDynamicSharedMemorySize, (int) dyn_lds));
   });
-  std::vector<uint64_t> go((size_t) ng + 1);
-  HIP_CHECK(hipMemcpyAsync(go.data(), goff, go.size() * 8, hipMemcpyDeviceToHost, st));
-  HIP_CHECK(hipStreamSynchronize(st));
-  uint64_t max_group = 0;
-  for (uint32_t g = 0; g < ng; ++g) max_group = std::max<uint64_t>(max_group, go[g + 1] - go[g]);
+  uint64_t max_group = std::min<uint64_t>(max_group_bound, n);
+  if (!max_group_bound)
+  {
+    std::vector<uint64_t> go((size_t) ng + 1);
+    HIP_CHECK(hipMemcpyAsync(go.data(), goff, go.size() * 8, hipMemcpyDeviceToHost, st));
+    HIP_CHECK(hipStreamSynchronize(st));
+    for (uint32_t g = 0; g < ng; ++g) max_group = std::max<uint64_t>(max_group, go[g + 1] - go[g]);
+  }
   const uint32_t n_wide = std::min<uint32_t>(SJ_MAX_WIDE, std::max<uint32_t>(1, cdiv(n, 1u << 16)));
   const uint32_t n_narrow = std::min<uint32_t>(SJ_MAX_NARROW, std::max<uint32_t>(1, cdiv(n, 1u << 16)));
   SjParams S = {};
@@ -1254,7 +1258,7 @@
   }
 }
 
-void std_sort_groups(uint32_t *key, uint32_t *idx, const uint32_t *gof, const uint64_t *goff, uint32_t ng, uint64_t n64, SortEmuBufs &b, hipStream_t st)
+void std_sort_groups(uint32_t *key, uint32_t *idx, const uint32_t *gof, const uint64_t *goff, uint32_t ng, uint64_t n64, SortEmuBufs &b, hipStream_t st, uint64_t max_group_bound)
 {
   if (n64 == 0 || ng == 0) return;
   if (n64 > 0x7FFFFFF0ull) throw bk_error(BK_ERR_LIMIT, "std_sort_groups: more than 2^31 pairs");
@@ -1306,7 +1310,7 @@
     }
     ++call;
   }
-  std_sort_groups_tasks(key, idx, gof, goff, ng, n, b, st, chk ? key0 : nullptr);
+  std_sort_groups_tasks(key, idx, gof, goff, ng, n, b, st, chk ? key0 : nullptr, max_group_bound);
 }
 static void window_sorts(uint32_t *key, uint32_t *idx, const uint32_t *gof, uint32_t n, hipStream_t st)
 {
```

Result: no change. 11800 (median of 6 runs) (+0.9%).
